# sidward14/gan-lab

Hardware: AMD Instinct MI355X
Metric: images/sec (G+D step), StyleGAN 1024^2 bs32/GPU (higher is better)
Workload: dtype f32; 1 GPU; StyleGAN res_samples=1024 FFHQ-shaped synthetic, bs=32/GPU fp32, nonsaturating + R1(lambda=10) + drift, stabilised phase, 1 D-iter + 1 G-iter; global_batch=32, per_gpu_batch=32, parallelism=single

## Files before the change

### gan_lab_amd/_lib.py

```python
import ctypes
import os
import subprocess

import torch

_HERE = os.path.dirname(os.path.abspath(__file__))
CSRC = os.path.join(_HERE, 'csrc')
SO_PATH = os.path.join(CSRC, os.path.basename(os.environ.get('GANLAB_HIP_LIB', '') or 'libganlab_hip.so'))

_c_int, _c_ll, _c_f, _c_p, _c_sz, _c_u64 = (ctypes.c_int, ctypes.c_longlong, ctypes.c_float, ctypes.c_void_p,
                                             ctypes.c_size_t, ctypes.c_uint64)
_c_d = ctypes.c_double

ACT_NONE, ACT_LRELU = 0, 1
PACK_FWD, PACK_DGRAD = 0, 1


class ConvGeom(ctypes.Structure):
    _fields_ = [('N', _c_int), ('Cin', _c_int), ('Hin', _c_int), ('Win', _c_int),
                ('Cout', _c_int), ('ks', _c_int), ('pad', _c_int), ('up', _c_int), ('pool', _c_int)]


_GP = ctypes.POINTER(ConvGeom)

# ... 1 lines not shown
class PackDesc(ctypes.Structure):
    _fields_ = [('src', _c_p), ('dst', _c_p), ('kind', _c_int), ('Cout', _c_int), ('Cin', _c_int), ('ks', _c_int),
                ('mode', _c_int), ('up', _c_int), ('scale', _c_f), ('reserved', _c_int), ('total', _c_ll),
                ('block0', _c_ll)]

class SnJob(ctypes.Structure):
    _fields_ = [('w', _c_p), ('w_sn', _c_p), ('g_sn', _c_p), ('gw', _c_p), ('u', _c_p), ('v', _c_p), ('sigma', _c_p),
                ('tpart', _c_p), ('s', _c_p), ('dpart', _c_p), ('R', _c_int), ('K', _c_int), ('blk_t0', _c_ll),
                ('blk_s0', _c_ll), ('blk_e0', _c_ll)]


SN_ROW_CHUNK, SN_COL_TILE, SN_ELEM_BLOCK = 16, 1024, 2048


class OrthoJob(ctypes.Structure):
    _fields_ = [('w', _c_p), ('gw', _c_p), ('s', _c_p), ('q', _c_p), ('part', _c_p), ('penalty', _c_p), ('R', _c_int),
                ('K', _c_int), ('form', _c_int), ('n_part', _c_int), ('blk_g0', _c_ll), ('blk_a0', _c_ll)]


class EwmaJob(ctypes.Structure):
    _fields_ = [('dst', _c_p), ('src', _c_p), ('count', _c_ll)]


ORTHO_TILE, ORTHO_QROWS, ORTHO_ROW, ORTHO_COL = 64, 4, 0, 1


class HierJob(ctypes.Structure):
    _fields_ = [('w', _c_p), ('gw', _c_p), ('gw_own', _c_p), ('C', _c_int), ('z_off', _c_int), ('z_len', _c_int),
                ('col', _c_int), ('scale', _c_f), ('one', _c_f), ('blk_f0', _c_ll), ('blk_w0', _c_ll)]


SIGNATURES = {
    'ganlab_abi_version': (_c_int, []),
    'ganlab_last_launch': (_c_int, [ctypes.c_char_p, _c_int, ctypes.POINTER(ctypes.c_uint)]),
    'ganlab_launch_count': (ctypes.c_ulonglong, []),
    'ganlab_launch_history': (_c_int, [_c_int, ctypes.c_char_p, _c_int, ctypes.POINTER(ctypes.c_uint)]),
    'ganlab_conv_geom_size': (_c_int, []),
    'ganlab_conv_out_hw': (_c_int, [_GP, ctypes.POINTER(_c_int), ctypes.POINTER(_c_int)]),
    'ganlab_conv_pack_f32': (_c_ll, [_c_p, _c_p, _c_int, _c_int, _c_int, _c_int, _c_f, _c_p]),
    'ganlab_conv_fwd_f32': (_c_int, [_c_p, _c_p, _c_p, _c_p, _GP, _c_f, _c_int, _c_f, _c_p]),
    'ganlab_conv_dgrad_f32': (_c_int, [_c_p, _c_p, _c_p, _GP, _c_p]),
    'ganlab_conv_splitk_plan': (_c_int, [_GP, _c_int]),
    'ganlab_conv_fwd_splitk_f32': (_c_int, [_c_p, _c_p, _c_p, _c_p, _GP, _c_f, _c_int, _c_f, _c_p, _c_sz, _c_p]),
    'ganlab_conv_dgrad_splitk_f32': (_c_int, [_c_p, _c_p, _c_p, _GP, _c_p, _c_sz, _c_p]),
    'ganlab_conv_dgrad_mask_supported': (_c_int, [_GP]),
    'ganlab_conv_dgrad_mask_f32': (_c_int, [_c_p, _c_p, _c_p, _c_p, _GP, _c_f, _c_p]),
    'ganlab_conv_act_bwd_fused_supported': (_c_int, [_GP]),
    'ganlab_conv_dgrad_act_f32': (_c_int, [_c_p, _c_p, _c_p, _c_p, _GP, _c_f, _c_p]),
    'ganlab_conv_fwd_mask_f32': (_c_int, [_c_p, _c_p, _c_p, _c_p, _GP, _c_f, _c_p]),
    'ganlab_conv_wgrad_act_f32': (_c_int, [_c_p, _c_p, _c_p, _c_p, _c_p, _GP, _c_f, _c_f, _c_f, _c_p, _c_sz, _c_p]),
    'ganlab_conv_wgrad_workspace': (_c_sz, [_GP]),
    'ganlab_conv_wgrad_f32': (_c_int, [_c_p, _c_p, _c_p, _GP, _c_f, _c_p, _c_sz, _c_p]),
    'ganlab_conv_s2_supported': (_c_int, [_GP]),
    'ganlab_conv_s2_pack_f32': (_c_ll, [_c_p, _c_p, _c_int, _c_int, _c_int, _c_int, _c_f, _c_p]),
    'ganlab_conv_s2_fwd_f32': (_c_int, [_c_p, _c_p, _c_p, _c_p, _GP, _c_f, _c_int, _c_f, _c_p]),
    'ganlab_conv_s2_dgrad_f32': (_c_int, [_c_p, _c_p, _c_p, _GP, _c_p]),
    'ganlab_conv_s2_wgrad_workspace': (_c_sz, [_GP]),
    'ganlab_conv_s2_wgrad_f32': (_c_int, [_c_p, _c_p, _c_p, _GP, _c_f, _c_p, _c_sz, _c_p]),
    'ganlab_conv_bf16_supported': (_c_int, [_GP]),
    'ganlab_conv_pack_bf16': (_c_ll, [_c_p, _c_p, _c_int, _c_int, _c_int, _c_f, _c_p]),
    'ganlab_conv_fwd_bf16': (_c_int, [_c_p, _c_p, _c_p, _c_p, _GP, _c_f, _c_int, _c_f, _c_p]),
    'ganlab_conv_dgrad_bf16': (_c_int, [_c_p, _c_p, _c_p, _GP, _c_p]),
    'ganlab_conv_bf16_splitk_plan': (_c_int, [_GP, _c_int]),
    'ganlab_conv_fwd_bf16_splitk': (_c_int, [_c_p, _c_p, _c_p, _c_p, _GP, _c_f, _c_int, _c_f, _c_p, _c_sz, _c_p]),
    'ganlab_conv_dgrad_bf16_splitk': (_c_int, [_c_p, _c_p, _c_p, _GP, _c_p, _c_sz, _c_p]),
    'ganlab_conv_wgrad_bf16_workspace': (_c_sz, [_GP]),
    'ganlab_conv_wgrad_bf16': (_c_int, [_c_p, _c_p, _c_p, _GP, _c_f, _c_p, _c_sz, _c_p]),
    'ganlab_conv_x3_supported': (_c_int, [_GP, _c_int]),
    'ganlab_conv_x3_pack': (_c_ll, [_c_p, _c_p, _c_int, _c_int, _c_int, _c_f, _c_p]),
    'ganlab_conv_fwd_x3': (_c_int, [_c_p, _c_p, _c_p, _c_p, _GP, _c_f, _c_int, _c_f, _c_p]),
    'ganlab_conv_dgrad_x3': (_c_int, [_c_p, _c_p, _c_p, _GP, _c_p]),
    'ganlab_conv_dgrad_mask_x3': (_c_int, [_c_p, _c_p, _c_p, _c_p, _GP, _c_f, _c_p]),
    'ganlab_conv_fwd_aff_x3': (_c_int, [_c_p, _c_p, _c_p, _c_p, _c_p, _c_p, _GP, _c_f, _c_int, _c_f, _c_p]),
    'ganlab_conv_fwd_aff_tail_x3_chunks': (_c_int, [_GP]),
    'ganlab_conv_s2_x3_supported': (_c_int, [_GP, _c_int]),
    'ganlab_conv_s2_x3_pack': (_c_ll, [_c_p, _c_p, _c_int, _c_int, _c_int, _c_f, _c_p]),
    'ganlab_conv_s2_fwd_x3': (_c_int, [_c_p, _c_p, _c_p, _c_p, _GP, _c_f, _c_int, _c_f, _c_p]),
    'ganlab_conv_s2_fwd_aff_x3': (_c_int, [_c_p, _c_p, _c_p, _c_p, _c_p, _c_p, _GP, _c_f, _c_int, _c_f, _c_p]),
    'ganlab_conv_s2_dgrad_x3': (_c_int, [_c_p, _c_p, _c_p, _GP, _c_p]),
    'ganlab_conv_s2_down_x3_supported': (_c_int, [_GP, _c_int]),
    'ganlab_conv_s2_down_x3_pack': (_c_ll, [_c_p, _c_p, _c_int, _c_int, _c_int, _c_f, _c_p]),
    'ganlab_conv_s2_down_fwd_x3': (_c_int, [_c_p, _c_p, _c_p, _c_p, _GP, _c_f, _c_int, _c_f, _c_p]),
    'ganlab_conv_s2_down_dgrad_x3': (_c_int, [_c_p, _c_p, _c_p, _GP, _c_p]),
    'ganlab_conv_wgrad_x3_supported': (_c_int, [_GP]),
    'ganlab_conv_wgrad_x3_workspace': (_c_sz, [_GP]),
    'ganlab_conv_wgrad_x3': (_c_int, [_c_p, _c_p, _c_p, _c_p, _c_p, _GP, _c_f, _c_p, _c_sz, _c_p]),
    'ganlab_conv_s2_wgrad_x3_supported': (_c_int, [_GP]),
    'ganlab_conv_s2_wgrad_x3_workspace': (_c_sz, [_GP]),
    'ganlab_conv_s2_wgrad_x3': (_c_int, [_c_p, _c_p, _c_p, _c_p, _c_p, _GP, _c_f, _c_p, _c_sz, _c_p]),
    'ganlab_conv_fwd_aff_tail_x3': (_c_int, [_c_p, _c_p, _c_p, _c_p, _c_p, _c_p, _c_p, _c_p, _c_p, _c_p, _GP, _c_f, _c_int, _c_f,
                                             _c_f, _c_p, _c_sz, _c_p]),
    'ganlab_mask_bits_supported': (_c_int, [_c_int, _c_int]),
    'ganlab_blur3x3_bits_f32': (_c_int, [_c_p, _c_p, _c_p, _c_ll, _c_int, _c_int, _c_p]),
    'ganlab_blur_act_bwd_bits_f32': (_c_int, [_c_p, _c_p, _c_p, _c_p, _c_int, _c_int, _c_int, _c_int, _c_f, _c_f,
                                              _c_p, _c_sz, _c_p]),
    'ganlab_act_bwd_blur_bits_f32': (_c_int, [_c_p, _c_p, _c_p, _c_p, _c_p, _c_p, _c_int, _c_int, _c_int, _c_int,
                                              _c_f, _c_f, _c_p, _c_sz, _c_p]),
    'ganlab_conv_fwd_blur_supported': (_c_int, [_GP, _c_p, _c_p]),
    'ganlab_conv_fwd_blur_bits_f32': (_c_int, [_c_p, _c_p, _c_p, _c_p, _c_p, _GP, _c_f, _c_f, _c_p]),
    'ganlab_conv_s2_blur_supported': (_c_int, [_GP]),
    'ganlab_conv_s2_blur_workspace': (_c_sz, [_GP]),
    'ganlab_conv_s2_fwd_blur_tail_f32': (_c_int, [_c_p, _c_p, _c_p, _c_p, _c_p, _c_p, _c_p, _c_p, _c_p, _c_p, _GP, _c_f, _c_int,
                                                  _c_f, _c_f, _c_p, _c_sz, _c_p]),
    'ganlab_conv_s2_dgrad_blur_act_bits_f32': (_c_int, [_c_p, _c_p, _c_p, _c_p, _c_p, _GP, _c_f, _c_f, _c_p, _c_sz, _c_p]),
    'ganlab_conv_dgrad_rgb_sums_supported': (_c_int, [_GP, _c_int]),
    'ganlab_conv_dgrad_rgb_sums_workspace': (_c_sz, [_GP]),
    'ganlab_conv_dgrad_rgb_sums_f32': (_c_int, [_c_p, _c_p, _c_p, _c_p, _c_p, _c_p, _GP, _c_int, _c_f, _c_f, _c_f, _c_int, _c_int,
                                                _c_p, _c_sz, _c_p]),
    'ganlab_conv_fwd_bits_f32': (_c_int, [_c_p, _c_p, _c_p, _c_p, _c_p, _GP, _c_f, _c_int, _c_f, _c_p]),
    'ganlab_conv_dgrad_act_bits_f32': (_c_int, [_c_p, _c_p, _c_p, _c_p, _GP, _c_f, _c_p]),
    'ganlab_conv_fwd_mask_bits_f32': (_c_int, [_c_p, _c_p, _c_p, _c_p, _GP, _c_f, _c_p]),
    'ganlab_conv_wgrad_act_bits_f32': (_c_int, [_c_p, _c_p, _c_p, _c_p, _c_p, _GP, _c_f, _c_f, _c_f, _c_p, _c_sz, _c_p]),
    'ganlab_pack_desc_size': (_c_int, []),
    'ganlab_pack_many': (_c_int, [_c_p, _c_int, _c_ll, _c_p]),
    'ganlab_in_affine_f32': (_c_int, [_c_p, _c_p, _c_p, _c_p, _c_p, _c_int, _c_int, _c_p]),
    'ganlab_conv_aff_supported': (_c_int, [_GP]),
    'ganlab_conv_fwd_aff_f32': (_c_int, [_c_p, _c_p, _c_p, _c_p, _c_p, _c_p, _GP, _c_f, _c_int, _c_f, _c_p]),
    'ganlab_conv_fwd_aff_tail_chunks': (_c_int, [_GP]),
    'ganlab_conv_fwd_aff_tail_f32': (_c_int, [_c_p, _c_p, _c_p, _c_p, _c_p, _c_p, _c_p, _c_p, _c_p, _c_p, _GP, _c_f, _c_int, _c_f,
                                              _c_f, _c_p, _c_sz, _c_p]),
    'ganlab_conv_wgrad_aff_f32': (_c_int, [_c_p, _c_p, _c_p, _c_p, _c_p, _GP, _c_f, _c_p, _c_sz, _c_p]),
    'ganlab_conv_s2_aff_supported': (_c_int, [_GP]),
    'ganlab_conv_s2_fwd_aff_f32': (_c_int, [_c_p, _c_p, _c_p, _c_p, _c_p, _c_p, _GP, _c_f, _c_int, _c_f, _c_p]),
    'ganlab_conv_s2_wgrad_aff_f32': (_c_int, [_c_p, _c_p, _c_p, _c_p, _c_p, _GP, _c_f, _c_p, _c_sz, _c_p]),
    'ganlab_mod_conv_supported': (_c_int, [_GP]),
    'ganlab_mod_conv_stat_chunks': (_c_int, [_GP]),
    'ganlab_mod_conv_fwd_f32': (_c_int, [_c_p, _c_p, _c_p, _c_p, _c_p, _c_p, _c_p, _c_p, _c_p, _c_p, _GP, _c_f, _c_int,
                                         _c_f, _c_f, _c_p, _c_sz, _c_p]),
    'ganlab_mod_torgb_prep_f32': (_c_int, [_c_p, _c_p, _c_p, _c_p, _c_p, _c_p, _c_int, _c_int, _c_int, _c_f, _c_f, _c_p]),
    'ganlab_mod_torgb_wgrad_f32': (_c_int, [_c_p, _c_p, _c_p, _c_p, _c_p, _c_int, _c_int, _c_int, _c_f, _c_f, _c_p]),
    'ganlab_mod_torgb_fwd_f32': (_c_int, [_c_p, _c_p, _c_p, _c_p, _c_int, _c_int, _c_int, _c_ll, _c_p]),
    'ganlab_mod_torgb_cross_workspace': (_c_sz, [_c_int]),
    'ganlab_mod_torgb_cross_f32': (_c_int, [_c_p, _c_p, _c_p, _c_int, _c_int, _c_int, _c_ll, _c_p, _c_sz, _c_p]),
    'ganlab_blur3x3_f32': (_c_int, [_c_p, _c_p, _c_ll, _c_int, _c_int, _c_p]),
    'ganlab_up2_f32': (_c_int, [_c_p, _c_p, _c_ll, _c_int, _c_int, _c_f, _c_p]),
    'ganlab_pool2_f32': (_c_int, [_c_p, _c_p, _c_ll, _c_int, _c_int, _c_f, _c_p]),
    'ganlab_resample2d_f32': (_c_int, [_c_p, _c_p, _c_p, _c_p, _c_p, _c_p, _c_ll, _c_int, _c_int, _c_int, _c_int, _c_int,
                                       _c_int, _c_p]),
    'ganlab_bias_act_f32': (_c_int, [_c_p, _c_p, _c_p, _c_p, _c_p, _c_int, _c_int, _c_ll, _c_f, _c_int, _c_f, _c_p]),
    'ganlab_act_bwd_f32': (_c_int, [_c_p, _c_p, _c_p, _c_ll, _c_f, _c_p]),
    'ganlab_act_bwd_bias_f32': (_c_int, [_c_p, _c_p, _c_p, _c_p, _c_int, _c_int, _c_ll, _c_f, _c_f, _c_p, _c_sz, _c_p]),
    'ganlab_channel_sum_f32': (_c_int, [_c_p, _c_p, _c_p, _c_int, _c_int, _c_ll, _c_f, _c_p, _c_sz, _c_p]),
    'ganlab_channel_sum_workspace': (_c_sz, [_c_int, _c_int, _c_ll]),
    'ganlab_instnorm_stats_f32': (_c_int, [_c_p, _c_p, _c_p, _c_ll, _c_ll, _c_f, _c_p]),
    'ganlab_row_stats_workspace': (_c_sz, [_c_ll, _c_ll]),
    'ganlab_row_stats_f32': (_c_int, [_c_p, _c_p, _c_p, _c_ll, _c_ll, _c_f, _c_p, _c_sz, _c_p]),
    'ganlab_instnorm_style_fwd_f32': (_c_int, [_c_p, _c_p, _c_p, _c_p, _c_p, _c_int, _c_int, _c_ll, _c_p]),
    'ganlab_instnorm_style_bwd_reduce_f32': (_c_int, [_c_p, _c_p, _c_p, _c_p, _c_p, _c_p, _c_ll, _c_ll, _c_p]),
    'ganlab_instnorm_style_bwd_apply_f32': (_c_int, [_c_p, _c_p, _c_p, _c_p, _c_p, _c_p, _c_p, _c_p, _c_int, _c_int,
                                                     _c_ll, _c_p]),
    'ganlab_pixelnorm_fwd_f32': (_c_int, [_c_p, _c_p, _c_int, _c_int, _c_ll, _c_f, _c_p]),
    'ganlab_pixelnorm_bwd_f32': (_c_int, [_c_p, _c_p, _c_p, _c_int, _c_int, _c_ll, _c_f, _c_p]),
    'ganlab_blur_fused_supported': (_c_int, [_c_int, _c_int]),
    'ganlab_blur_fused_workspace': (_c_sz, [_c_int, _c_int, _c_int, _c_int]),
    'ganlab_blur_bias_act_f32': (_c_int, [_c_p, _c_p, _c_p, _c_p, _c_p, _c_int, _c_int, _c_int, _c_int, _c_f,
                                          _c_int, _c_f, _c_p]),
    'ganlab_blur_act_bwd_f32': (_c_int, [_c_p, _c_p, _c_p, _c_p, _c_int, _c_int, _c_int, _c_int, _c_f, _c_f,
                                         _c_p, _c_sz, _c_p]),
    'ganlab_act_bwd_blur_f32': (_c_int, [_c_p, _c_p, _c_p, _c_p, _c_p, _c_p, _c_int, _c_int, _c_int, _c_int,
                                         _c_f, _c_f, _c_p, _c_sz, _c_p]),
    'ganlab_act_stats_workspace': (_c_sz, [_c_int, _c_int, _c_ll]),
    'ganlab_bias_act_stats_f32': (_c_int, [_c_p, _c_p, _c_p, _c_p, _c_p, _c_p, _c_p, _c_int, _c_int, _c_ll, _c_f, _c_int,
                                           _c_f, _c_f, _c_p, _c_sz, _c_p]),
    'ganlab_blur_bias_act_stats_f32': (_c_int, [_c_p, _c_p, _c_p, _c_p, _c_p, _c_p, _c_p, _c_int, _c_int, _c_int, _c_int,
                                                _c_f, _c_int, _c_f, _c_f, _c_p, _c_sz, _c_p]),
    'ganlab_instnorm_bwd_act_workspace': (_c_sz, [_c_int, _c_int, _c_ll]),
    'ganlab_instnorm_style_bwd_act_f32': (_c_int, [_c_p] * 11 + [_c_int, _c_int, _c_ll, _c_int, _c_f, _c_f, _c_p, _c_sz,
                                                                 _c_p]),
    'ganlab_instnorm_bwd_rgb_supported': (_c_int, [_c_int, _c_int, _c_int, _c_ll]),
    'ganlab_instnorm_bwd_reduce_rgb_workspace': (_c_sz, [_c_int, _c_int, _c_ll]),
    'ganlab_instnorm_style_bwd_reduce_rgb_f32': (_c_int, [_c_p, _c_p, _c_int] + [_c_p] * 5 + [_c_int, _c_int, _c_ll, _c_p,
                                                                                            _c_sz, _c_p]),
    'ganlab_instnorm_style_bwd_act_rgb_f32': (_c_int, [_c_p, _c_p, _c_int] + [_c_p] * 10 + [_c_int, _c_int, _c_ll, _c_int,
                                                                                         _c_f, _c_f, _c_p, _c_sz, _c_p]),
    'ganlab_instnorm_style_bwd_act_blur_f32': (_c_int, [_c_p] * 11 + [_c_int, _c_int, _c_int, _c_int, _c_int, _c_f, _c_f,
                                                                      _c_p, _c_sz, _c_p]),
    'ganlab_u8_box_decode_f32': (_c_int, [_c_p, _c_p, _c_int, _c_int, _c_int, _c_int, _c_int, _c_p, _c_p, _c_p, _c_p]),
    'ganlab_chan_affine_f32': (_c_int, [_c_p, _c_p, _c_p, _c_p, _c_int, _c_int, _c_ll, _c_p]),
    'ganlab_mul_f32': (_c_int, [_c_p, _c_p, _c_p, _c_ll, _c_p]),
    'ganlab_ln_affine_fwd_f32': (_c_int, [_c_p, _c_p, _c_p, _c_p, _c_p, _c_p, _c_int, _c_ll, _c_int, _c_f, _c_p]),
    'ganlab_colscale_f32': (_c_int, [_c_p, _c_p, _c_p, _c_int, _c_ll, _c_p]),
    'ganlab_coldot_f32': (_c_int, [_c_p, _c_p, _c_p, _c_p, _c_p, _c_p, _c_int, _c_ll, _c_p]),
    'ganlab_ln_rowsums_workspace': (_c_sz, [_c_int, _c_ll]),
    'ganlab_ln_rowsums_f32': (_c_int, [_c_p, _c_p, _c_p, _c_p, _c_p, _c_p, _c_p, _c_p, _c_int, _c_ll, _c_p, _c_sz, _c_p, _c_p,
                                       _c_f, _c_p]),
    'ganlab_ln_project_f32': (_c_int, [_c_p, _c_p, _c_p, _c_p, _c_p, _c_p, _c_p, _c_p, _c_int, _c_ll, _c_p]),
    'ganlab_ln_bwd_cols_f32': (_c_int, [_c_p, _c_p, _c_p, _c_p, _c_p, _c_p, _c_p, _c_p, _c_p, _c_int, _c_ll, _c_p]),
    'ganlab_ln_bwdbwd_apply_f32': (_c_int, [_c_p, _c_p, _c_p, _c_p, _c_p, _c_p, _c_p, _c_p, _c_int, _c_ll, _c_p]),
    'ganlab_bn_stats_f32': (_c_int, [_c_p, _c_p, _c_int, _c_int, _c_ll, _c_p, _c_sz, _c_p]),
    'ganlab_bn_finalize_f32': (_c_int, [_c_p, _c_p, _c_p, _c_p, _c_p, _c_p, _c_int, _c_f, _c_f, _c_f, _c_p]),
    'ganlab_bn_apply_f32': (_c_int, [_c_p, _c_p, _c_p, _c_p, _c_p, _c_int, _c_int, _c_ll, _c_int, _c_f, _c_p]),
    'ganlab_bn_bwd_sums_f32': (_c_int, [_c_p, _c_p, _c_p, _c_p, _c_p, _c_int, _c_int, _c_ll, _c_p, _c_sz, _c_p, _c_p, _c_f,
                                        _c_p]),
    'ganlab_bn_bwd_apply_f32': (_c_int, [_c_p, _c_p, _c_p, _c_p, _c_p, _c_p, _c_p, _c_int, _c_int, _c_ll, _c_p]),
    'ganlab_tanh_fwd_f32': (_c_int, [_c_p, _c_p, _c_ll, _c_p]),
    'ganlab_tanh_bwd_f32': (_c_int, [_c_p, _c_p, _c_p, _c_ll, _c_p]),
    'ganlab_mbstd_fwd_f32': (_c_int, [_c_p, _c_p, _c_int, _c_int, _c_ll, _c_f, _c_p]),
    'ganlab_mbstd_bwd_f32': (_c_int, [_c_p, _c_p, _c_p, _c_int, _c_int, _c_ll, _c_f, _c_p]),
    'ganlab_mbstd_bwdbwd_f32': (_c_int, [_c_p, _c_p, _c_p, _c_p, _c_p, _c_int, _c_int, _c_ll, _c_f, _c_p]),
    'ganlab_axpby_f32': (_c_int, [_c_p, _c_p, _c_p, _c_ll, _c_f, _c_f, _c_p]),
    'ganlab_scale_dev_f32': (_c_int, [_c_p, _c_p, _c_p, _c_ll, _c_f, _c_p]),
    'ganlab_lerp_rows_f32': (_c_int, [_c_p, _c_p, _c_p, _c_p, _c_ll, _c_ll, _c_p]),
    'ganlab_sum_f32': (_c_int, [_c_p, _c_p, _c_ll, _c_f, _c_int, _c_p, _c_sz, _c_p]),
    'ganlab_sum_workspace': (_c_sz, [_c_ll]),
    'ganlab_bce_logits_fwd_f32': (_c_int, [_c_p, _c_p, _c_int, _c_f, _c_p]),
    'ganlab_bce_logits_bwd_f32': (_c_int, [_c_p, _c_p, _c_p, _c_int, _c_f, _c_p]),
    'ganlab_hinge_fwd_f32': (_c_int, [_c_p, _c_p, _c_int, _c_f, _c_f, _c_p]),
    'ganlab_hinge_bwd_f32': (_c_int, [_c_p, _c_p, _c_p, _c_int, _c_f, _c_f, _c_p]),
    'ganlab_chnorm_penalty_fwd_f32': (_c_int, [_c_p, _c_p, _c_int, _c_int, _c_ll, _c_f, _c_f, _c_p, _c_sz, _c_p]),
    'ganlab_chnorm_penalty_bwd_f32': (_c_int, [_c_p, _c_p, _c_p, _c_int, _c_int, _c_ll, _c_f, _c_f, _c_p]),
    'ganlab_adam_f32': (_c_int, [_c_p, _c_p, _c_p, _c_p, _c_ll, _c_f, _c_f, _c_f, _c_f, _c_f, _c_f, _c_f, _c_p]),
    'ganlab_ewma_f32': (_c_int, [_c_p, _c_p, _c_ll, _c_f, _c_p]),
    'ganlab_randn_f32': (_c_int, [_c_p, _c_ll, _c_u64, _c_u64, _c_p]),
    'ganlab_randn_dev_f32': (_c_int, [_c_p, _c_ll, _c_u64, _c_p, _c_u64, _c_p]),
    'ganlab_diffaug_params_f32': (_c_int, [_c_p, _c_int, _c_int, _c_int, _c_u64, _c_u64, _c_p]),
    'ganlab_diffaug_params_dev_f32': (_c_int, [_c_p, _c_int, _c_int, _c_int, _c_u64, _c_p, _c_u64, _c_p]),
    'ganlab_diffaug_fwd_workspace': (_c_sz, [_c_int, _c_int, _c_int, _c_int]),
    'ganlab_diffaug_bwd_workspace': (_c_sz, [_c_int, _c_int, _c_int, _c_int]),
    'ganlab_diffaug_fwd_f32': (_c_int, [_c_p, _c_p, _c_p, _c_int, _c_int, _c_int, _c_int, _c_p, _c_sz, _c_p]),
    'ganlab_diffaug_bwd_f32': (_c_int, [_c_p, _c_p, _c_p, _c_int, _c_int, _c_int, _c_int, _c_p, _c_sz, _c_p]),
    'ganlab_ada_params_f32': (_c_int, [_c_p, _c_int, _c_int, _c_int, _c_p, _c_int, _c_u64, _c_u64, _c_p]),
    'ganlab_ada_params_dev_f32': (_c_int, [_c_p, _c_int, _c_int, _c_int, _c_p, _c_int, _c_u64, _c_p, _c_u64, _c_p]),
    'ganlab_ada_fwd_f32': (_c_int, [_c_p, _c_p, _c_p, _c_int, _c_int, _c_int, _c_p]),
    'ganlab_ada_bwd_f32': (_c_int, [_c_p, _c_p, _c_p, _c_int, _c_int, _c_int, _c_p]),
    'ganlab_ada_update_f32': (_c_int, [_c_p, _c_p, _c_int, _c_int, _c_f, _c_f, _c_p]),
    'ganlab_ada_filter_bank': (_c_int, [_c_p]),
    'ganlab_ada_ext_params_f32': (_c_int, [_c_p, _c_int, _c_int, _c_int, _c_p, _c_int, _c_u64, _c_u64, _c_p]),
    'ganlab_ada_ext_params_dev_f32': (_c_int, [_c_p, _c_int, _c_int, _c_int, _c_p, _c_int, _c_u64, _c_p, _c_u64, _c_p]),
    'ganlab_ada_ext_fwd_f32': (_c_int, [_c_p, _c_p, _c_p, _c_p, _c_int, _c_int, _c_int, _c_p]),
    'ganlab_ada_ext_bwd_f32': (_c_int, [_c_p, _c_p, _c_p, _c_int, _c_int, _c_int, _c_p]),
    'ganlab_swd_down_f32': (_c_int, [_c_p, _c_p, _c_ll, _c_int, _c_int, _c_p]),
    'ganlab_swd_band_f32': (_c_int, [_c_p, _c_p, _c_p, _c_ll, _c_int, _c_int, _c_p]),
    'ganlab_swd_gather_f32': (_c_int, [_c_p, _c_p, _c_p, _c_p, _c_int, _c_int, _c_int, _c_p]),
    'ganlab_swd_stats_f64': (_c_int, [_c_p, _c_ll, _c_ll, _c_p, _c_p]),
    'ganlab_swd_project_f32': (_c_int, [_c_p, _c_p, _c_p, _c_p, _c_ll, _c_int, _c_p]),
    'ganlab_swd_sort_workspace': (_c_sz, [_c_int, _c_ll]),
    'ganlab_swd_sort_f32': (_c_int, [_c_p, _c_p, _c_int, _c_ll, _c_p, _c_sz, _c_p]),
    'ganlab_swd_distance_workspace': (_c_sz, [_c_int, _c_ll]),
    'ganlab_swd_distance_f64': (_c_int, [_c_p, _c_p, _c_p, _c_int, _c_ll, _c_p, _c_sz, _c_p]),
    'ganlab_swd_positions_i32': (_c_int, [_c_p, _c_int, _c_int, _c_int, _c_u64, _c_u64, _c_p]),
    'ganlab_swd_directions_f32': (_c_int, [_c_p, _c_int, _c_u64, _c_u64, _c_p]),
    'ganlab_msssim_workspace': (_c_sz, [_c_int, _c_int]),
    'ganlab_msssim_level_f32': (_c_int, [_c_p, _c_p, _c_ll, _c_p, _c_p, _c_ll, _c_int, _c_int, _c_int, _c_int, _c_int, _c_f, _c_f,
                                         _c_p, _c_sz, _c_p]),
    'ganlab_msssim_finish_f64': (_c_int, [_c_p, _c_sz, _c_int, _c_int, _c_p, _c_p, _c_p, _c_p]),
    'ganlab_spectrum_workspace': (_c_sz, [_c_int, _c_int]),
    'ganlab_spectrum_scratch': (_c_sz, [_c_int, _c_int]),
    'ganlab_spectrum_feed_f32': (_c_int, [_c_p, _c_ll, _c_int, _c_int, _c_int, _c_int, _c_int, _c_p, _c_sz, _c_p, _c_sz, _c_p]),
    'ganlab_spectrum_finish_f64': (_c_int, [_c_p, _c_p, _c_sz, _c_int, _c_int, _c_p, _c_sz, _c_p]),
    'ganlab_adam_dev_f32': (_c_int, [_c_p, _c_p, _c_p, _c_p, _c_ll, _c_p, _c_f, _c_f, _c_f, _c_f, _c_p]),
    'ganlab_sn_job_size': (_c_int, []),
    'ganlab_sn_refresh': (_c_int, [_c_p, _c_int, _c_ll, _c_ll, _c_ll, _c_int, _c_f, _c_p]),
    'ganlab_sn_backward': (_c_int, [_c_p, _c_int, _c_ll, _c_p]),
    'ganlab_ortho_job_size': (_c_int, []),
    'ganlab_ortho_apply': (_c_int, [_c_p, _c_int, _c_ll, _c_ll, _c_f, _c_p, _c_p]),
    'ganlab_attn_supported': (_c_int, [_c_int, _c_int, _c_int, _c_int, _c_int]),
    'ganlab_attn_fwd_f32': (_c_int, [_c_p, _c_p, _c_p, _c_p, _c_p, _c_int, _c_int, _c_int, _c_int, _c_int, _c_p]),
    'ganlab_attn_bwd_workspace': (_c_sz, [_c_int, _c_int]),
    'ganlab_attn_bwd_f32': (_c_int, [_c_p] * 9 + [_c_int, _c_int, _c_int, _c_int, _c_int, _c_p, _c_sz, _c_p]),
    'ganlab_maxpool2x2_bits_bytes': (_c_sz, [_c_ll, _c_int, _c_int]),
    'ganlab_maxpool2x2_f32': (_c_int, [_c_p, _c_p, _c_p, _c_ll, _c_int, _c_int, _c_p]),
    'ganlab_maxpool2x2_bwd_f32': (_c_int, [_c_p, _c_p, _c_p, _c_ll, _c_int, _c_int, _c_p]),
    'ganlab_gated_residual_f32': (_c_int, [_c_p, _c_p, _c_p, _c_p, _c_ll, _c_p]),
    'ganlab_dot_workspace': (_c_sz, [_c_ll]),
    'ganlab_dot_f32': (_c_int, [_c_p, _c_p, _c_p, _c_ll, _c_p, _c_sz, _c_p]),
    'ganlab_cbn_apply_f32': (_c_int, [_c_p] * 7 + [_c_int, _c_int, _c_ll, _c_int, _c_int, _c_f, _c_p]),
    'ganlab_cbn_bwd_workspace': (_c_sz, [_c_int, _c_int]),
    'ganlab_cbn_bwd_f32': (_c_int, [_c_p] * 12 + [_c_int, _c_int, _c_ll, _c_int, _c_int, _c_f, _c_p, _c_sz, _c_p]),
    'ganlab_hier_job_size': (_c_int, []),
    'ganlab_hier_fwd_f32': (_c_int, [_c_p, _c_int, _c_ll, _c_p, _c_p, _c_p, _c_p, _c_int, _c_ll, _c_int, _c_int, _c_int, _c_p]),
    'ganlab_hier_bwd_f32': (_c_int, [_c_p, _c_int, _c_ll] + [_c_p] * 7 + [_c_int, _c_ll, _c_int, _c_int, _c_int, _c_int, _c_p]),
    'ganlab_trunc_randn_f32': (_c_int, [_c_p, _c_ll, _c_f, _c_u64, _c_u64, _c_p]),
    'ganlab_ewma_job_size': (_c_int, []),
    'ganlab_ewma_many_f32': (_c_int, [_c_p, _c_int, _c_f, _c_p]),
    'ganlab_mbn_apply_f32': (_c_int, [_c_p, _c_p, _c_p, _c_p, _c_ll, _c_p, _c_ll, _c_p, _c_int, _c_int, _c_ll, _c_int, _c_f,
                                      _c_p]),
    'ganlab_mbn_bwd_workspace': (_c_sz, [_c_int, _c_int]),
    'ganlab_mbn_bwd_f32': (_c_int, [_c_p] * 5 + [_c_ll] + [_c_p] * 5 + [_c_ll, _c_p, _c_int, _c_int, _c_ll, _c_int, _c_f, _c_p,
                                    _c_sz, _c_p]),
    'ganlab_proj_fwd_f32': (_c_int, [_c_p, _c_p, _c_p, _c_p, _c_p, _c_int, _c_ll, _c_int, _c_p]),
    'ganlab_proj_dfeat_f32': (_c_int, [_c_p, _c_p, _c_p, _c_p, _c_int, _c_ll, _c_int, _c_p]),
    'ganlab_proj_dweight_f32': (_c_int, [_c_p, _c_p, _c_p, _c_p, _c_int, _c_ll, _c_int, _c_p]),
    'ganlab_randint_i32': (_c_int, [_c_p, _c_ll, _c_int, _c_u64, _c_u64, _c_p]),
    'ganlab_prdc_norms_f32': (_c_int, [_c_p, _c_p, _c_ll, _c_int, _c_p]),
    'ganlab_prdc_knn_f32': (_c_int, [_c_p, _c_p, _c_p, _c_ll, _c_int, _c_int, _c_p]),
    'ganlab_prdc_cross_f32': (_c_int, [_c_p] * 5 + [_c_int, _c_p, _c_p, _c_p, _c_ll, _c_ll, _c_int, _c_p]),
    'ganlab_cr_params_i32': (_c_int, [_c_p, _c_int, _c_int, _c_int, _c_u64, _c_u64, _c_p, _c_p]),
    'ganlab_cr_transform_f32': (_c_int, [_c_p, _c_p, _c_p, _c_int, _c_int, _c_int, _c_int, _c_p]),
    'ganlab_cr_msd_fwd_f32': (_c_int, [_c_p, _c_p, _c_p, _c_int, _c_p]),
    'ganlab_cr_msd_bwd_f32': (_c_int, [_c_p, _c_p, _c_p, _c_p, _c_p, _c_int, _c_p]),
    'ganlab_cr_imsd_workspace': (_c_sz, [_c_ll]),
    'ganlab_cr_imsd_fwd_f32': (_c_int, [_c_p, _c_p, _c_p, _c_ll, _c_p, _c_sz, _c_p]),
    'ganlab_cr_imsd_bwd_f32': (_c_int, [_c_p, _c_p, _c_p, _c_p, _c_p, _c_ll, _c_p]),
    'ganlab_moments_accum_f32': (_c_int, [_c_p, _c_ll, _c_int, _c_p, _c_p, _c_p, _c_p]),
    'ganlab_kid_rowsums_f32': (_c_int, [_c_p, _c_ll, _c_p, _c_ll, _c_int, _c_f, _c_f, _c_int, _c_p, _c_p]),
    'ganlab_class_ce_fwd_f32': (_c_int, [_c_p, _c_p, _c_p, _c_p, _c_int, _c_int, _c_p]),
    'ganlab_class_ce_bwd_f32': (_c_int, [_c_p, _c_p, _c_p, _c_p, _c_p, _c_int, _c_int, _c_p]),
    'ganlab_cl_supported': (_c_int, [_c_int, _c_int, _c_int]),
    'ganlab_cl_fwd_f32': (_c_int, [_c_p] * 5 + [_c_int, _c_int, _c_int, _c_int, _c_f, _c_f, _c_f, _c_p]),
    'ganlab_cl_bwd_workspace': (_c_sz, [_c_int, _c_int, _c_int]),
    'ganlab_cl_bwd_f32': (_c_int, [_c_p] * 7 + [_c_int, _c_int, _c_int, _c_int, _c_f, _c_f, _c_f, _c_p, _c_sz, _c_p]),
    'ganlab_pyramid_mse_workspace': (_c_sz, [_c_int, _c_int, _c_int, _c_int]),
    'ganlab_pyramid_mse_f32': (_c_int, [_c_p] * 3 + [_c_int] + [_c_p] * 3 + [_c_int, _c_int, _c_int, _c_p, _c_sz, _c_p]),
    'ganlab_scale_rows_f32': (_c_int, [_c_p, _c_p, _c_p, _c_int, _c_ll, _c_p]),
    'ganlab_w_moments_workspace': (_c_sz, [_c_int]),
    'ganlab_w_moments_f32': (_c_int, [_c_p, _c_p, _c_p, _c_ll, _c_int, _c_p, _c_sz, _c_p]),
    'ganlab_project_step_f32': (_c_int, [_c_p] * 8 + [_c_int, _c_int, _c_int, _c_int, _c_p, _c_p]),
    'ganlab_step_scalars_size': (_c_int, []),
    'ganlab_set_step_scalars': (_c_int, [_c_p, _c_u64, _c_f, _c_f, _c_f, _c_f, _c_f, _c_f, _c_p]),
    'ganlab_ppl_endpoints_f32': (_c_int, [_c_p, _c_p, _c_p, _c_p, _c_ll, _c_int, _c_d, _c_int, _c_int, _c_u64, _c_u64, _c_p]),
    'ganlab_row_sqdist_f32': (_c_int, [_c_p, _c_p, _c_p, _c_ll, _c_ll, _c_p]),
    'ganlab_trimmed_mean_workspace': (_c_sz, [_c_ll]),
    'ganlab_trimmed_mean_f32': (_c_int, [_c_p, _c_ll, _c_d, _c_d, _c_p, _c_p, _c_sz, _c_p]),
}

_LIB = None


class GanlabLibraryError(RuntimeError):
    pass


def build(verbose=False):
    res = subprocess.run(['make', '-C', CSRC, '-j4'], capture_output=True, text=True)
    if verbose or res.returncode != 0:
        print(res.stdout)
        print(res.stderr)
    if res.returncode != 0:
        raise GanlabLibraryError('building libganlab_hip.so failed:\n' + res.stderr[-4000:])
    return SO_PATH


def lib():
    global _LIB
    if _LIB is None:
        if not os.path.exists(SO_PATH):
            raise GanlabLibraryError(
                f'{SO_PATH} not found: the HIP kernel library is required (there is no CPU/PyTorch '
                f'fallback). Build it with `python -c "import __graft_entry__ as g; g.build()"` or '
                f'`make -C {CSRC}`.')
        handle = ctypes.CDLL(SO_PATH)
        for name, (res, args) in SIGNATURES.items():
            fn = getattr(handle, name)
            fn.restype = res
            fn.argtypes = args
        if handle.ganlab_conv_geom_size() != ctypes.sizeof(ConvGeom):
            raise GanlabLibraryError(f'ConvGeom mirror is {ctypes.sizeof(ConvGeom)} bytes, the library\'s '
                                     f'ganlab_conv_geom {handle.ganlab_conv_geom_size()}: header and binding disagree')
        if handle.ganlab_pack_desc_size() != ctypes.sizeof(PackDesc):
            raise GanlabLibraryError(f'PackDesc mirror is {ctypes.sizeof(PackDesc)} bytes, the library\'s '
                                     f'ganlab_pack_desc {handle.ganlab_pack_desc_size()}: header and binding disagree')
        if handle.ganlab_sn_job_size() != ctypes.sizeof(SnJob):
            raise GanlabLibraryError(f'SnJob mirror is {ctypes.sizeof(SnJob)} bytes, the library\'s '
                                     f'ganlab_sn_job {handle.ganlab_sn_job_size()}: header and binding disagree')
        if handle.ganlab_ortho_job_size() != ctypes.sizeof(OrthoJob):
            raise GanlabLibraryError(f'OrthoJob mirror is {ctypes.sizeof(OrthoJob)} bytes, the library\'s '
                                     f'ganlab_ortho_job {handle.ganlab_ortho_job_size()}: header and binding disagree')
        if handle.ganlab_hier_job_size() != ctypes.sizeof(HierJob):
            raise GanlabLibraryError(f'HierJob mirror is {ctypes.sizeof(HierJob)} bytes, the library\'s '
                                     f'ganlab_hier_job {handle.ganlab_hier_job_size()}: header and binding disagree')
        if handle.ganlab_ewma_job_size() != ctypes.sizeof(EwmaJob):
            raise GanlabLibraryError(f'EwmaJob mirror is {ctypes.sizeof(EwmaJob)} bytes, the library\'s '
                                     f'ganlab_ewma_job {handle.ganlab_ewma_job_size()}: header and binding disagree')
        _LIB = handle
    return _LIB


def last_launch():
    buf = ctypes.create_string_buffer(1024)
    grid = ctypes.c_uint(0)
    n = lib().ganlab_last_launch(buf, 1024, ctypes.byref(grid))
    return (buf.value.decode() if n > 0 else None), int(grid.value)


def launch_count():
    return int(lib().ganlab_launch_count())


def launches_since(count):
    n = min(launch_count() - count, 16)
    out = []
    buf = ctypes.create_string_buffer(1024)
    grid = ctypes.c_uint(0)
    for back in range(n - 1, -1, -1):
        if lib().ganlab_launch_history(back, buf, 1024, ctypes.byref(grid)) > 0:
            out.append((buf.value.decode(), int(grid.value)))
    return out


_ERR = {-1: 'GANLAB_EINVAL (bad argument)', -2: 'GANLAB_EWORKSPACE (workspace too small)',
        -3: 'GANLAB_ELAUNCH (kernel launch failed)', -4: 'GANLAB_EUNSUPPORTED (geometry not handled)'}


def check(rc, what):
    if rc != 0:
        raise GanlabLibraryError(f'{what} failed: {_ERR.get(rc, rc)}')
```

### gan_lab_amd/_ops/pointwise.py

```python
import numpy as np

import torch
from torch.autograd import Function
from torch.autograd.function import once_differentiable

from .. import _lib
from .._lib import check
from .core import _c, _nchw, _new, _p, _st, _take


def k_blur(x):
    x = _c(x)
    n, c, h, w = x.shape
    y = torch.empty_like(x)
    check(_lib.lib().ganlab_blur3x3_f32(_p(x), _p(y), n * c, h, w, _st()), 'blur3x3')
    return y


def decode_u8(images_u8_nhwc, res, mean, std, flip=None):
    x = images_u8_nhwc
    if not x.is_cuda or x.dtype != torch.uint8 or x.dim() != 4:
        raise TypeError('decode_u8 needs a (N,H,W,C) uint8 tensor on the GPU')
    x = x.contiguous()
    n, hs, ws, c = x.shape
    if hs % res or ws % res or hs // res != ws // res:
        raise ValueError(f'cannot box-resize {hs}x{ws} to {res}x{res}')
    mean = torch.as_tensor(mean, dtype=torch.float32, device=x.device).contiguous()
    std = torch.as_tensor(std, dtype=torch.float32, device=x.device).contiguous()
    assert mean.numel() == c and std.numel() == c
    if flip is not None:
        flip = flip.to(device=x.device, dtype=torch.uint8).contiguous()
        assert flip.numel() == n
    out = torch.empty((n, c, res, res), dtype=torch.float32, device=x.device)
    check(_lib.lib().ganlab_u8_box_decode_f32(x.data_ptr(), _p(out), n, hs, ws, c, hs // res, _p(mean), _p(std),
                                              flip.data_ptr() if flip is not None else None, _st()), 'u8_box_decode')
    return out


def k_up2(x, scale=1.0):
    x = _c(x)
    n, c, h, w = x.shape
    y = _new((n, c, 2 * h, 2 * w), x)
    check(_lib.lib().ganlab_up2_f32(_p(x), _p(y), n * c, h, w, scale, _st()), 'up2')
    return y


def k_pool2(x, scale=0.25):
    x = _c(x)
    n, c, h, w = x.shape
    assert h % 2 == 0 and w % 2 == 0
    y = _new((n, c, h // 2, w // 2), x)
    check(_lib.lib().ganlab_pool2_f32(_p(x), _p(y), n * c, h // 2, w // 2, scale, _st()), 'pool2')
    return y


RESAMPLE_MODES = ('bilinear_up', 'bilinear_down', 'nearest_down')


_RESAMPLE_TABLES = {}


def resample_matrix(mode, align_corners, n_in):
    if mode not in RESAMPLE_MODES:
        raise ValueError(f'resampler mode {mode!r}: one of {RESAMPLE_MODES}')
    f32 = np.float32
    n_out = 2 * n_in if mode == 'bilinear_up' else n_in // 2
    if n_out < 1 or (mode != 'bilinear_up' and n_in % 2):
        raise ValueError(f'{mode}: size {n_in} has no 0.5x / 2x counterpart')
    m = np.zeros((n_out, n_in), np.float64)
    inv = f32(0.5) if mode == 'bilinear_up' else f32(2.0)
    for o in range(n_out):
        if mode == 'nearest_down':
            m[o, min(int(np.floor(f32(o) * inv)), n_in - 1)] = 1.0
            continue
        if align_corners:
            r = f32(n_in - 1) / f32(n_out - 1) if n_out > 1 else f32(0)
            src = r * f32(o)
        else:
            src = max(inv * (f32(o) + f32(0.5)) - f32(0.5), f32(0))
        i0 = min(int(src), n_in - 1)
        i1 = i0 + (1 if i0 < n_in - 1 else 0)
        l1 = f32(src) - f32(i0)
        m[o, i0] += float(f32(1) - l1)
        m[o, i1] += float(l1)
    return m


def _taps(m):
    nz = [np.nonzero(row)[0] for row in m]
    t = max(1, max(len(v) for v in nz))
    if t > 6:
        raise ValueError(f'resampler needs {t} taps per output (the kernel holds 6)')
    idx, w = np.zeros((m.shape[0], t), np.int32), np.zeros((m.shape[0], t), np.float32)
    for o, v in enumerate(nz):
        idx[o, :len(v)] = v
        w[o, :len(v)] = m[o, v]
    return idx, w, t


def _resample_tables(mode, align, n_in, adjoint, device):
    key = (mode, bool(align), int(n_in), bool(adjoint), str(device))
    tab = _RESAMPLE_TABLES.get(key)
    if tab is None:
        m = resample_matrix(mode, align, n_in)
        idx, w, t = _taps(m.T if adjoint else m)
        tab = (torch.from_numpy(idx).to(device), torch.from_numpy(w).to(device), t, idx.shape[0])
        _RESAMPLE_TABLES[key] = tab
    return tab


def k_resample(x, mode, align, hin, win, adjoint):
    x = _c(x)
    n, c, h, w = x.shape
    iy, wy, ty, ho = _resample_tables(mode, align, hin, adjoint, x.device)
    ix, wx, tx, wo = _resample_tables(mode, align, win, adjoint, x.device)
    exp_h = hin if not adjoint else (2 * hin if mode == 'bilinear_up' else hin // 2)
    exp_w = win if not adjoint else (2 * win if mode == 'bilinear_up' else win // 2)
    if (h, w) != (exp_h, exp_w):
        raise ValueError(f'resample {mode} (adjoint={adjoint}): input {h}x{w}, expected {exp_h}x{exp_w}')
    y = _new((n, c, ho, wo), x)
    check(_lib.lib().ganlab_resample2d_f32(_p(x), _p(y), _p(iy), _p(wy), _p(ix), _p(wx), n * c, h, w, ho, wo, ty, tx,
                                           _st()), 'resample2d')
    return y


def k_bias_act(x, bias, noise, noise_w, bias_scale, act, slope):
    x = _c(x)
    n, c, hw = _nchw(x)
    y = torch.empty_like(x)
    bias = _c(bias) if bias is not None else None
    noise = _c(noise) if noise is not None else None
    noise_w = _c(noise_w) if noise_w is not None else None
    if noise is not None:
        assert noise.numel() == n * hw and noise_w.numel() == c
    check(_lib.lib().ganlab_bias_act_f32(_p(x), _p(bias), _p(noise), _p(noise_w), _p(y), n, c, hw, bias_scale, act,
                                         slope, _st()), 'bias_act')
    return y


def k_act_bwd(gy, y, slope):
    gy, y = _c(gy), _c(y)
    assert gy.shape == y.shape
    gz = torch.empty_like(gy)
    check(_lib.lib().ganlab_act_bwd_f32(_p(gy), _p(y), _p(gz), gy.numel(), slope, _st()), 'act_bwd')
    return gz


def k_act_bwd_bias(gy, y, slope, scale):
    gy, y = _c(gy), _c(y)
    assert gy.shape == y.shape
    n, c, hw = _nchw(gy)
    L = _lib.lib()
    ws = torch.empty((L.ganlab_channel_sum_workspace(n, c, hw) + 3) // 4, dtype=torch.float32, device=gy.device)
    gz, gb = torch.empty_like(gy), _take('gb', (c,), gy)
    check(L.ganlab_act_bwd_bias_f32(_p(gy), _p(y), _p(gz), _p(gb), n, c, hw, slope, scale, _p(ws), ws.numel() * 4,
                                    _st()), 'act_bwd_bias')
    return gz, gb


def k_channel_sum(a, b=None, scale=1.0, sink=None):
    a = _c(a)
# ... 331 lines not shown
```

### gan_lab_amd/csrc/pointwise.hip

```cpp
#include "common.h"

#include <stdlib.h>

namespace {

constexpr int kMaxBlocks = 256 * 8;

inline unsigned ew_blocks(long long n_items) {
  long long b = (n_items + 255) / 256;
  if (b < 1) b = 1;
  if (b > kMaxBlocks) b = kMaxBlocks;
  return (unsigned)b;
}

struct ChunkRange { long long begin, end, stride; };
__device__ __forceinline__ ChunkRange chunk_range(long long hw4, int chunks, int c, int contig) {
  ChunkRange r;
  if (contig) {
    const long long rows = (hw4 + 255) / 256, per = (rows + chunks - 1) / chunks;
    r.begin = (long long)c * per * 256;
    r.end = r.begin + per * 256;
    if (r.end > hw4) r.end = hw4;
    r.stride = 256;
  } else {
    r.begin = (long long)c * 256;
    r.end = hw4;
    r.stride = (long long)chunks * 256;
  }
  return r;
}
inline int pw_contig() {
  static const int v = [] { const char* e = getenv("GANLAB_PW_CONTIG"); return (e && e[0] == '0') ? 0 : 1; }();
  return v;
}

#define GRID_STRIDE(i, n) \
  for (long long i = blockIdx.x * (long long)blockDim.x + threadIdx.x; i < (n); i += (long long)gridDim.x * blockDim.x)

__global__ void blur3x3_kernel(const float* __restrict__ x, float* __restrict__ y, long long planes, int H, int W) {
  const long long total = planes * H * W;
  GRID_STRIDE(i, total) {
    const int w = (int)(i % W);
    const long long t = i / W;
    const int h = (int)(t % H);
    const float* px = x + (t - h) * W;
    float acc = 0.f;
#pragma unroll
    for (int dy = -1; dy <= 1; ++dy) {
      const int yy = h + dy;
      if ((unsigned)yy >= (unsigned)H) continue;
      const float* row = px + (long long)yy * W;
      const float l = (w > 0) ? row[w - 1] : 0.f;
      const float c = row[w];
      const float r = (w + 1 < W) ? row[w + 1] : 0.f;
      const float rs = l + 2.f * c + r;
      acc += (dy == 0) ? 2.f * rs : rs;
    }
    y[i] = acc * (1.f / 16.f);
  }
}

__device__ __forceinline__ unsigned mask_nibble(const unsigned* __restrict__ bits, long long e) {
  return (bits[e >> 5] >> (unsigned)(e & 31)) & 0xFu;
}
__device__ __forceinline__ unsigned mask_bit(const unsigned* __restrict__ bits, long long e) {
  return (bits[e >> 5] >> (unsigned)(e & 31)) & 1u;
}

template <bool MASKED, bool BITS = false>
__device__ __forceinline__ void blur_row(const float* __restrict__ in, const float* __restrict__ m, long long ro,
                                         int x0, int q, int w4, bool valid, float slope, float (&hrow)[4],
                                         float (&cen)[4], const unsigned* __restrict__ mb = nullptr,
                                         long long mplane = 0) {
  float4 v = make_float4(0.f, 0.f, 0.f, 0.f);
  if (valid) {
    v = *reinterpret_cast<const float4*>(in + ro + x0);
    if (MASKED) {
      if (BITS) {
        const unsigned nb = mask_nibble(mb, mplane + ro + x0);
        v.x = (nb & 1u) ? v.x : v.x * slope;
        v.y = (nb & 2u) ? v.y : v.y * slope;
        v.z = (nb & 4u) ? v.z : v.z * slope;
        v.w = (nb & 8u) ? v.w : v.w * slope;
      } else {
        const float4 mm = *reinterpret_cast<const float4*>(m + ro + x0);
        v.x = mm.x > 0.f ? v.x : v.x * slope;
        v.y = mm.y > 0.f ? v.y : v.y * slope;
        v.z = mm.z > 0.f ? v.z : v.z * slope;
        v.w = mm.w > 0.f ? v.w : v.w * slope;
      }
    }
  }
  const int lane = threadIdx.x & 63;
  float l = __shfl_up(v.w, 1, 64);
  float r = __shfl_down(v.x, 1, 64);
  const bool need_l = lane == 0 && q != 0, need_r = lane == 63 && q != w4 - 1;
  float e = 0.f;
  if (valid && (need_l || need_r)) {
    const long long eo = ro + x0 + (need_l ? -1 : 4);
    e = in[eo];
    if (MASKED) {
      if (BITS) e = mask_bit(mb, mplane + eo) ? e : e * slope;
      else e = m[eo] > 0.f ? e : e * slope;
    }
  }
  if (q == 0) l = 0.f;
  else if (lane == 0) l = e;
  if (q == w4 - 1) r = 0.f;
  else if (lane == 63) r = e;
  hrow[0] = l + 2.f * v.x + v.y;
  hrow[1] = v.x + 2.f * v.y + v.z;
  hrow[2] = v.y + 2.f * v.z + v.w;
  hrow[3] = v.z + 2.f * v.w + r;
  cen[0] = v.x; cen[1] = v.y; cen[2] = v.z; cen[3] = v.w;
}

template <int R, bool BITS = false>
__global__ __launch_bounds__(256) void blur3x3_vec_kernel(const float* __restrict__ x, float* __restrict__ y,
                                                          long long planes, int H, int W,
                                                          unsigned* __restrict__ bits = nullptr) {
  const int w4 = W >> 2, hr = H / R;
  const long long total = planes * hr * w4;
  const long long span = (long long)gridDim.x * blockDim.x;
  for (long long base = blockIdx.x * (long long)blockDim.x; base < total; base += span) {
    const long long i = base + threadIdx.x;
    const bool live = i < total;
    const long long ii = live ? i : total - 1;
    const int q = (int)(ii % w4);
    const long long t = ii / w4;
    const int rr = (int)(t % hr);
    const long long pl = t / hr;
    const float* px = x + pl * H * W;
    const int y0 = R * rr, x0 = 4 * q;
    float h[R + 2][4], cen[4];
    [[maybe_unused]] unsigned nib[R];
#pragma unroll
    for (int k = 0; k < R + 2; ++k) {
      const int yy = y0 - 1 + k;
      blur_row<false>(px, nullptr, (long long)yy * W, x0, q, w4, (unsigned)yy < (unsigned)H, 0.f, h[k], cen);
      if constexpr (BITS) {
        if (k >= 1 && k <= R)
          nib[k - 1] = (cen[0] > 0.f ? 1u : 0u) | (cen[1] > 0.f ? 2u : 0u) | (cen[2] > 0.f ? 4u : 0u) | (cen[3] > 0.f ? 8u : 0u);
      }
    }
    if constexpr (BITS) {
      const int sh = 4 * (threadIdx.x & 7);
#pragma unroll
      for (int k = 0; k < R; ++k) {
        unsigned wv = nib[k] << sh;
        wv |= __shfl_xor(wv, 1, 64);
        wv |= __shfl_xor(wv, 2, 64);
        wv |= __shfl_xor(wv, 4, 64);
        if (live && (threadIdx.x & 7) == 0) bits[(pl * H * W + (long long)(y0 + k) * W + x0) >> 5] = wv;
      }
    }
    if (live) {
      float* py = y + pl * H * W + (long long)y0 * W + x0;
#pragma unroll
      for (int k = 0; k < R; ++k) {
        float4 o;
        o.x = (h[k][0] + 2.f * h[k + 1][0] + h[k + 2][0]) * 0.0625f;
        o.y = (h[k][1] + 2.f * h[k + 1][1] + h[k + 2][1]) * 0.0625f;
        o.z = (h[k][2] + 2.f * h[k + 1][2] + h[k + 2][2]) * 0.0625f;
        o.w = (h[k][3] + 2.f * h[k + 1][3] + h[k + 2][3]) * 0.0625f;
        *reinterpret_cast<float4*>(py + (long long)k * W) = o;
      }
    }
  }
}

__global__ void up2_kernel(const float* __restrict__ x, float* __restrict__ y, long long planes, int H, int W,
                           float scale) {
  const int Wo = 2 * W, Ho = 2 * H;
  const long long total = planes * Ho * Wo;
  GRID_STRIDE(i, total) {
    const int w = (int)(i % Wo);
    const long long t = i / Wo;
    const int h = (int)(t % Ho);
    const long long pl = t / Ho;
    y[i] = scale * x[(pl * H + (h >> 1)) * W + (w >> 1)];
  }
}

__global__ void pool2_kernel(const float* __restrict__ x, float* __restrict__ y, long long planes, int Ho, int Wo,
                             float scale) {
  const int W = 2 * Wo;
  const long long total = planes * Ho * Wo;
  GRID_STRIDE(i, total) {
    const int w = (int)(i % Wo);
    const long long t = i / Wo;
    const float2 a = *reinterpret_cast<const float2*>(x + (2 * t) * W + 2 * w);
    const float2 b = *reinterpret_cast<const float2*>(x + (2 * t + 1) * W + 2 * w);
    y[i] = scale * ((a.x + a.y) + (b.x + b.y));
  }
}

enum { BF_FWD = 0, BF_A = 1, BF_AT = 2 };

template <int MODE, int R, bool STATS = false, bool BITS = false>
__global__ __launch_bounds__(256) void blur_fused_kernel(const float* __restrict__ in, const float* __restrict__ y,
                                                         const float* __restrict__ noise,
                                                         const float* __restrict__ bias,
                                                         const float* __restrict__ noise_w, float* __restrict__ out,
                                                         double* __restrict__ part, int N, int C, int H, int W,
                                                         int chunks, float bias_scale, int act, float slope,
                                                         int want_sums, double* __restrict__ spart = nullptr) {
  __shared__ double red[4];
  __shared__ double dred[2][4];
  const int c = blockIdx.y, chunk = blockIdx.x;
  const int w4 = W >> 2, hr = H / R;
  const long long per_n = (long long)hr * w4, total = STATS ? per_n : (long long)N * per_n, HW = (long long)H * W;
  double ds = 0.0, dss = 0.0;
  const float b = (MODE == BF_FWD && bias) ? bias[c] * bias_scale : 0.f;
  const float nw = (MODE == BF_FWD && noise) ? noise_w[c] : 0.f;
  double s0 = 0.0, s1 = 0.0;
  for (long long base = chunk * 256LL; base < total; base += (long long)chunks * 256) {
    const long long i = base + threadIdx.x;
    const bool live = i < total;
    const long long ii = live ? i : total - 1;
    const long long n = STATS ? (long long)blockIdx.z : ii / per_n, rem = STATS ? ii : ii - n * per_n;
    const int rr = (int)(rem / w4), q = (int)(rem - (long long)rr * w4);
    const long long plane = (n * C + c) * HW;
    const int y0 = R * rr, x0 = 4 * q;
    float h[R + 2][4], cen[R + 2][4];
#pragma unroll
    for (int k = 0; k < R + 2; ++k) {
      const int yy = y0 - 1 + k;
      blur_row<MODE == BF_AT, BITS>(in + plane, (MODE == BF_AT && !BITS) ? y + plane : nullptr, (long long)yy * W, x0, q,
                                    w4, (unsigned)yy < (unsigned)H, slope, h[k], cen[k],
                                    reinterpret_cast<const unsigned*>(y), plane);
    }
    if (!live) continue;
    const long long co = (long long)y0 * W + x0;
#pragma unroll
    for (int k = 0; k < R; ++k) {
      float o[4];
#pragma unroll
      for (int j = 0; j < 4; ++j) o[j] = (h[k][j] + 2.f * h[k + 1][j] + h[k + 2][j]) * 0.0625f;
      if (MODE == BF_FWD) {
        float nz[4] = {0.f, 0.f, 0.f, 0.f};
        if (noise) *reinterpret_cast<float4*>(nz) = *reinterpret_cast<const float4*>(noise + n * HW + co + k * W);
#pragma unroll
        for (int j = 0; j < 4; ++j) {
          float t = o[j] + b + nw * nz[j];
          if (act == GANLAB_ACT_LRELU) t = gl_lrelu(t, slope);
          o[j] = t;
          if (STATS) {
            const double d = (double)t;
            ds += d;
            dss += d * d;
          }
        }
      } else if (MODE == BF_A) {
        if constexpr (BITS) {
          const unsigned nb = mask_nibble(reinterpret_cast<const unsigned*>(y), plane + co + (long long)k * W);
#pragma unroll
          for (int j = 0; j < 4; ++j) {
            o[j] = ((nb >> j) & 1u) ? o[j] : o[j] * slope;
            s0 += (double)o[j];
          }
        } else {
          float m[4];
          *reinterpret_cast<float4*>(m) = *reinterpret_cast<const float4*>(y + plane + co + k * W);
#pragma unroll
          for (int j = 0; j < 4; ++j) {
            o[j] = m[j] > 0.f ? o[j] : o[j] * slope;
            s0 += (double)o[j];
          }
        }
      } else {
        float nz[4] = {0.f, 0.f, 0.f, 0.f};
        if (noise && want_sums)
          *reinterpret_cast<float4*>(nz) = *reinterpret_cast<const float4*>(noise + n * HW + co + k * W);
#pragma unroll
        for (int j = 0; j < 4; ++j) {
          s0 += (double)cen[k + 1][j];
          s1 += (double)cen[k + 1][j] * nz[j];
        }
      }
      *reinterpret_cast<float4*>(out + plane + co + (long long)k * W) = *reinterpret_cast<float4*>(o);
    }
  }
  if (STATS) {
#pragma unroll
    for (int o = 32; o > 0; o >>= 1) {
      ds += __shfl_xor(ds, o, 64);
      dss += __shfl_xor(dss, o, 64);
    }
    if ((threadIdx.x & 63) == 0) {
      dred[0][threadIdx.x >> 6] = ds;
      dred[1][threadIdx.x >> 6] = dss;
    }
    __syncthreads();
    if (threadIdx.x < 2) {
      const int k = threadIdx.x;
      spart[(((long long)blockIdx.z * C + c) * chunks + chunk) * 2 + k] = (dred[k][0] + dred[k][1]) + (dred[k][2] + dred[k][3]);
    }
  }
  if (MODE != BF_FWD && want_sums) {
    s0 = gl_block_sum_256d(s0, red);
    if (threadIdx.x == 0) part[(long long)c * chunks + chunk] = s0;
    if (MODE == BF_AT) {
      __syncthreads();
      s1 = gl_block_sum_256d(s1, red);
      if (threadIdx.x == 0) part[((long long)C + c) * chunks + chunk] = s1;
    }
  }
}

template <int R>
__global__ __launch_bounds__(256) void instnorm_bwd_act_blur_kernel(
    const float* __restrict__ gy, const float* __restrict__ x, const float* __restrict__ mean,
    const float* __restrict__ rstd, const float* __restrict__ style, const float* __restrict__ s1,
    const float* __restrict__ s2, const float* __restrict__ noise, float* __restrict__ out, double* __restrict__ part,
    int N, int C, int H, int W, int chunks, int act, float slope, int want_b, int want_nw) {
  __shared__ double red[4];
  const int c = blockIdx.y, n = blockIdx.z, chunk = blockIdx.x;
  const long long pl = (long long)n * C + c, HW = (long long)H * W;
  const int w4 = W >> 2, hr = H / R;
  const long long per_n = (long long)hr * w4;
  const double md = (double)mean[pl], rd = (double)rstd[pl];
  const double ys = style ? (double)style[((long long)n * 2 + 0) * C + c] + 1.0 : 1.0;
  const double inv = 1.0 / (double)HW;
  const double k = rd * ys, a1 = (double)s1[pl] * inv, a2 = (double)s2[pl] * inv;
  const float* pg = gy + pl * HW;
  const float* px = x + pl * HW;
  const float* pn = (want_nw && noise) ? noise + (long long)n * HW : nullptr;
  float* po = out + pl * HW;
  const int lane = threadIdx.x & 63;
  double sb = 0.0, snw = 0.0;
  auto zval = [&](float g, float v) -> double {
    double t = k * ((double)g - a1 - ((double)v - md) * rd * a2);
    if (act == GANLAB_ACT_LRELU && !(v > 0.f)) t *= (double)slope;
    return t;
  };
  for (long long base = chunk * 256LL; base < per_n; base += (long long)chunks * 256) {
    const long long i = base + threadIdx.x;
    const bool live = i < per_n;
    const long long ii = live ? i : per_n - 1;
    const int rr = (int)(ii / w4), q = (int)(ii - (long long)rr * w4);
    const int y0 = R * rr, x0 = 4 * q;
    float h[R + 2][4];
#pragma unroll
    for (int kk = 0; kk < R + 2; ++kk) {
      const int yy = y0 - 1 + kk;
      const bool valid = (unsigned)yy < (unsigned)H;
      const long long ro = (long long)yy * W;
      float z[4] = {0.f, 0.f, 0.f, 0.f};
      if (valid) {
        float g[4], v[4];
        *reinterpret_cast<float4*>(g) = *reinterpret_cast<const float4*>(pg + ro + x0);
        *reinterpret_cast<float4*>(v) = *reinterpret_cast<const float4*>(px + ro + x0);
        const bool own = live && kk >= 1 && kk <= R;
        float nz[4] = {0.f, 0.f, 0.f, 0.f};
        if (own && pn) *reinterpret_cast<float4*>(nz) = *reinterpret_cast<const float4*>(pn + ro + x0);
#pragma unroll
        for (int j = 0; j < 4; ++j) {
          const double t = zval(g[j], v[j]);
          z[j] = (float)t;
          if (own) {
            sb += t;
            snw += t * (double)nz[j];
          }
        }
      }
      float l = __shfl_up(z[3], 1, 64);
      float r = __shfl_down(z[0], 1, 64);
      const bool need_l = lane == 0 && q != 0, need_r = lane == 63 && q != w4 - 1;
      float e = 0.f;
      if (valid && (need_l || need_r)) {
        const long long eo = ro + x0 + (need_l ? -1 : 4);
        e = (float)zval(pg[eo], px[eo]);
      }
      if (q == 0) l = 0.f;
      else if (lane == 0) l = e;
      if (q == w4 - 1) r = 0.f;
      else if (lane == 63) r = e;
      h[kk][0] = l + 2.f * z[0] + z[1];
      h[kk][1] = z[0] + 2.f * z[1] + z[2];
      h[kk][2] = z[1] + 2.f * z[2] + z[3];
      h[kk][3] = z[2] + 2.f * z[3] + r;
    }
    if (!live) continue;
#pragma unroll
    for (int kk = 0; kk < R; ++kk) {
      float4 o;
      o.x = (h[kk][0] + 2.f * h[kk + 1][0] + h[kk + 2][0]) * 0.0625f;
      o.y = (h[kk][1] + 2.f * h[kk + 1][1] + h[kk + 2][1]) * 0.0625f;
      o.z = (h[kk][2] + 2.f * h[kk + 1][2] + h[kk + 2][2]) * 0.0625f;
      o.w = (h[kk][3] + 2.f * h[kk + 1][3] + h[kk + 2][3]) * 0.0625f;
      *reinterpret_cast<float4*>(po + (long long)(y0 + kk) * W + x0) = o;
    }
  }
  const long long slot = ((long long)c * N + n) * chunks + chunk;
  if (want_b) {
    sb = gl_block_sum_256d(sb, red);
    if (threadIdx.x == 0) part[slot] = sb;
  }
  if (want_nw) {
    if (want_b) __syncthreads();
    snw = gl_block_sum_256d(snw, red);
    if (threadIdx.x == 0) part[(long long)C * N * chunks + slot] = snw;
  }
}

inline int blur_rows(int H) { return (H & 3) == 0 ? 4 : 2; }
inline int blur_rows_mode(int H, int mode) {
  const int min8 = mode == BF_FWD ? 512 : (mode == BF_A ? 256 : (1 << 30));
  return ((H & 7) == 0 && H >= min8) ? 8 : blur_rows(H);
}
#define BLUR_FUSED_LAUNCH(MODE, ...)                                                                   \
  do {                                                                                                 \
    const int rows_ = blur_rows_mode(H, MODE);                                                         \
    if (rows_ == 8) GL_LAUNCH((blur_fused_kernel<MODE, 8>), dim3(chunks, C), dim3(256), 0, ST, __VA_ARGS__);      \
    else if (rows_ == 4) GL_LAUNCH((blur_fused_kernel<MODE, 4>), dim3(chunks, C), dim3(256), 0, ST, __VA_ARGS__); \
    else GL_LAUNCH((blur_fused_kernel<MODE, 2>), dim3(chunks, C), dim3(256), 0, ST, __VA_ARGS__);                \
  } while (0)

#define BLUR_FUSED_LAUNCH_BITS(MODE, ...)                                                                            \
  do {                                                                                                               \
    const int rows_ = blur_rows_mode(H, MODE);                                                                       \
    if (rows_ == 8) GL_LAUNCH((blur_fused_kernel<MODE, 8, false, true>), dim3(chunks, C), dim3(256), 0, ST, __VA_ARGS__);      \
    else if (rows_ == 4) GL_LAUNCH((blur_fused_kernel<MODE, 4, false, true>), dim3(chunks, C), dim3(256), 0, ST, __VA_ARGS__); \
    else GL_LAUNCH((blur_fused_kernel<MODE, 2, false, true>), dim3(chunks, C), dim3(256), 0, ST, __VA_ARGS__);                \
  } while (0)

inline int blur_fused_chunks(int N, int H, int W) {
  long long c = ((long long)N * (H / blur_rows(H)) * (W / 4) + 256 * 4 - 1) / (256 * 4);
  if (c < 1) c = 1;
  if (c > 128) c = 128;
  return (int)c;
}

__global__ __launch_bounds__(256) void bias_act_stats_kernel(const float* __restrict__ x, const float* __restrict__ bias,
                                                             const float* __restrict__ noise,
                                                             const float* __restrict__ noise_w, float* __restrict__ y,
                                                             double* __restrict__ spart, int C, long long hw4,
                                                             int chunks, float bias_scale, int act, float slope,
                                                             int contig) {
  __shared__ double dred[2][4];
  const long long pl = blockIdx.y;
  const int c = (int)(pl % C);
  const long long n = pl / C;
  const float b = bias ? bias[c] * bias_scale : 0.f;
  const float nw = noise ? noise_w[c] : 0.f;
  const float4* xp = reinterpret_cast<const float4*>(x) + pl * hw4;
  const float4* np = noise ? reinterpret_cast<const float4*>(noise) + n * hw4 : nullptr;
  float4* yp = reinterpret_cast<float4*>(y) + pl * hw4;
  double ds = 0.0, dss = 0.0;
  const ChunkRange cr = chunk_range(hw4, chunks, blockIdx.x, contig);
  for (long long i = cr.begin + threadIdx.x; i < cr.end; i += cr.stride) {
    float v[4], nz[4] = {0.f, 0.f, 0.f, 0.f};
    *reinterpret_cast<float4*>(v) = xp[i];
    if (np) *reinterpret_cast<float4*>(nz) = np[i];
#pragma unroll
    for (int k = 0; k < 4; ++k) {
      float t = v[k] + b + nw * nz[k];
      if (act == GANLAB_ACT_LRELU) t = gl_lrelu(t, slope);
      v[k] = t;
      const double d = (double)t;
      ds += d;
      dss += d * d;
    }
    yp[i] = *reinterpret_cast<float4*>(v);
  }
#pragma unroll
  for (int o = 32; o > 0; o >>= 1) {
    ds += __shfl_xor(ds, o, 64);
    dss += __shfl_xor(dss, o, 64);
  }
  if ((threadIdx.x & 63) == 0) {
    dred[0][threadIdx.x >> 6] = ds;
    dred[1][threadIdx.x >> 6] = dss;
  }
  __syncthreads();
  if (threadIdx.x < 2) {
    const int k = threadIdx.x;
    spart[(pl * chunks + blockIdx.x) * 2 + k] = (dred[k][0] + dred[k][1]) + (dred[k][2] + dred[k][3]);
  }
}

__global__ void act_stats_finish_kernel(const double* __restrict__ spart, float* __restrict__ mean,
                                        float* __restrict__ rstd, long long planes, int chunks, double inv_hw, float eps) {
  const long long pl = blockIdx.x * (long long)blockDim.x + threadIdx.x;
  if (pl >= planes) return;
  double s = 0.0, ss = 0.0;
  for (int k = 0; k < chunks; ++k) {
    s += spart[(pl * chunks + k) * 2];
    ss += spart[(pl * chunks + k) * 2 + 1];
  }
  const double m = s * inv_hw;
  double var = ss * inv_hw - m * m;
  if (var < 0.0) var = 0.0;
  mean[pl] = (float)m;
  rstd[pl] = (float)(1.0 / sqrt(var + (double)eps));
}

__global__ __launch_bounds__(256) void row_stats_partial_kernel(const float* __restrict__ x, double* __restrict__ spart,
                                                                int chunks, long long m4) {
  __shared__ double red[2][4];
  const long long row = blockIdx.x / chunks;
  const int k = blockIdx.x % chunks;
  const long long per = (m4 + chunks - 1) / chunks, lo = k * per, hi = lo + per < m4 ? lo + per : m4;
  const float4* p4 = reinterpret_cast<const float4*>(x) + row * m4;
  double s = 0.0, ss = 0.0;
  for (long long i = lo + threadIdx.x; i < hi; i += 256) {
    const float4 v = p4[i];
    const double a = (double)v.x, b = (double)v.y, c = (double)v.z, d = (double)v.w;
    s += (a + b) + (c + d);
    ss += (a * a + b * b) + (c * c + d * d);
  }
#pragma unroll
  for (int o = 32; o > 0; o >>= 1) {
    s += __shfl_xor(s, o, 64);
    ss += __shfl_xor(ss, o, 64);
  }
  if ((threadIdx.x & 63) == 0) {
    red[0][threadIdx.x >> 6] = s;
    red[1][threadIdx.x >> 6] = ss;
  }
  __syncthreads();
  if (threadIdx.x == 0) {
    spart[((long long)blockIdx.x) * 2] = (red[0][0] + red[0][1]) + (red[0][2] + red[0][3]);
    spart[((long long)blockIdx.x) * 2 + 1] = (red[1][0] + red[1][1]) + (red[1][2] + red[1][3]);
  }
}

inline int act_stats_chunks(long long hw4) {
  long long c = (hw4 + 256 * 8 - 1) / (256 * 8);
  if (c < 1) c = 1;
  if (c > 64) c = 64;
  return (int)c;
}

template <int VEC>
__global__ void bias_act_kernel(const float* __restrict__ x, const float* __restrict__ bias,
                                const float* __restrict__ noise, const float* __restrict__ noise_w,
                                float* __restrict__ y, int N, int C, long long HW, float bias_scale, int act,
                                float slope) {
  const long long hwv = HW / VEC, total = (long long)N * C * hwv;
  GRID_STRIDE(i, total) {
    const long long pl = i / hwv, hv = i - pl * hwv;
    const int c = (int)(pl % C);
    const long long n = pl / C;
    const float b = bias ? bias[c] * bias_scale : 0.f;
    const float nw = noise ? noise_w[c] : 0.f;
    float v[VEC], nz[VEC];
    if (VEC == 4) {
      *reinterpret_cast<float4*>(v) = *reinterpret_cast<const float4*>(x + i * 4);
      if (noise) *reinterpret_cast<float4*>(nz) = *reinterpret_cast<const float4*>(noise + (n * hwv + hv) * 4);
    } else {
      v[0] = x[i];
      if (noise) nz[0] = noise[n * HW + hv];
    }
#pragma unroll
    for (int k = 0; k < VEC; ++k) {
      float t = v[k] + b;
      if (noise) t += nw * nz[k];
      if (act == GANLAB_ACT_LRELU) t = gl_lrelu(t, slope);
      v[k] = t;
    }
    if (VEC == 4) *reinterpret_cast<float4*>(y + i * 4) = *reinterpret_cast<float4*>(v);
    else y[i] = v[0];
  }
}

__global__ void act_bwd_kernel(const float* __restrict__ gy, const float* __restrict__ y, float* __restrict__ gz,
                               long long n, long long n4, float slope) {
  GRID_STRIDE(i, n4) {
    const float4 g = reinterpret_cast<const float4*>(gy)[i];
    const float4 o = reinterpret_cast<const float4*>(y)[i];
    float4 r;
    r.x = o.x > 0.f ? g.x : g.x * slope;
    r.y = o.y > 0.f ? g.y : g.y * slope;
    r.z = o.z > 0.f ? g.z : g.z * slope;
    r.w = o.w > 0.f ? g.w : g.w * slope;
    reinterpret_cast<float4*>(gz)[i] = r;
  }
// ... 803 lines not shown
  __shared__ float red[4];
  double s = 0.0;
  for (int i = threadIdx.x; i < nb; i += 256) s += part[i];
  float f = gl_block_sum_256((float)s, red);
  if (threadIdx.x == 0) out[0] = f * scale;
}

inline int sum_blocks(long long n) {
  long long b = (n + 256 * 16 - 1) / (256 * 16);
  if (b < 1) b = 1;
  if (b > 1024) b = 1024;
  return (int)b;
}

__global__ __launch_bounds__(256) void bce_fwd_kernel(const float* __restrict__ x, float* __restrict__ out, int n,
                                                      float t) {
  __shared__ float red[4];
  float s = 0.f;
  for (int i = threadIdx.x; i < n; i += 256) {
    const float v = x[i];
    s += fmaxf(v, 0.f) - v * t + log1pf(expf(-fabsf(v)));
  }
  s = gl_block_sum_256(s, red);
  if (threadIdx.x == 0) out[0] = s / (float)n;
}

__global__ void bce_bwd_kernel(const float* __restrict__ x, const float* __restrict__ gout, float* __restrict__ gx,
                               int n, float t) {
  const int i = blockIdx.x * blockDim.x + threadIdx.x;
  if (i < n) {
    const float v = x[i];
    const float sg = 1.f / (1.f + expf(-v));
    gx[i] = gout[0] * (sg - t) / (float)n;
  }
}

__global__ __launch_bounds__(256) void hinge_fwd_kernel(const float* __restrict__ x, float* __restrict__ out, int n,
                                                        float a, float b) {
  __shared__ float red[4];
  float s = 0.f;
  for (int i = threadIdx.x; i < n; i += 256) s += fmaxf(a + b * x[i], 0.f);
  s = gl_block_sum_256(s, red);
  if (threadIdx.x == 0) out[0] = s / (float)n;
}

__global__ void hinge_bwd_kernel(const float* __restrict__ x, const float* __restrict__ gout, float* __restrict__ gx,
                                 int n, float a, float b) {
  const int i = blockIdx.x * blockDim.x + threadIdx.x;
  if (i < n) gx[i] = (a + b * x[i] > 0.f) ? gout[0] * b / (float)n : 0.f;
}

__global__ __launch_bounds__(256) void chnorm_pen_stage1(const float* __restrict__ g, float* __restrict__ part,
                                                         int N, int C, long long HW, float gamma) {
  __shared__ float red[4];
  const long long total = (long long)N * HW;
  float s = 0.f;
  GRID_STRIDE(i, total) {
    const long long n = i / HW, hw = i - n * HW;
    const float* p = g + n * C * HW + hw;
    float q = 0.f;
    for (int c = 0; c < C; ++c) q += p[c * HW] * p[c * HW];
    const float d = sqrtf(q) - gamma;
    s += d * d;
  }
  s = gl_block_sum_256(s, red);
  if (threadIdx.x == 0) part[blockIdx.x] = s;
}

__global__ void chnorm_pen_bwd_kernel(const float* __restrict__ g, const float* __restrict__ gout,
                                      float* __restrict__ gg, int N, int C, long long HW, float gamma, float scale) {
  const long long total = (long long)N * HW;
  const float go = gout[0] * scale * 2.f;
  GRID_STRIDE(i, total) {
    const long long n = i / HW, hw = i - n * HW;
    const float* p = g + n * C * HW + hw;
    float q = 0.f;
    for (int c = 0; c < C; ++c) q += p[c * HW] * p[c * HW];
    const float s = sqrtf(q);
    const float k = s > 0.f ? go * (s - gamma) / s : 0.f;
    float* o = gg + n * C * HW + hw;
    for (int c = 0; c < C; ++c) o[c * HW] = k * p[c * HW];
  }
}

__global__ void adam_kernel(float* __restrict__ p, const float* __restrict__ g, float* __restrict__ m,
                            float* __restrict__ v, long long n, float lr, float b1, float b2, float eps, float wd,
                            float bc1, float bc2, const float* __restrict__ dev) {
  if (dev != nullptr) {
    lr = dev[0];
    bc1 = dev[1];
    bc2 = dev[2];
  }
  const float step = lr / bc1, isq = rsqrtf(bc2);
  GRID_STRIDE(i, n) {
    float gi = g[i];
    const float pi = p[i];
    if (wd != 0.f) gi += wd * pi;
    const float mi = b1 * m[i] + (1.f - b1) * gi;
    const float vi = b2 * v[i] + (1.f - b2) * gi * gi;
    m[i] = mi;
    v[i] = vi;
    p[i] = pi - step * mi / (sqrtf(vi) * isq + eps);
  }
}

__global__ void ewma_kernel(float* __restrict__ lag, const float* __restrict__ p, long long n, float beta) {
  GRID_STRIDE(i, n) lag[i] = p[i] * (1.f - beta) + lag[i] * beta;
}

__global__ void randn_kernel(float* __restrict__ out, long long n, uint64_t seed, uint64_t offset,
                             const uint64_t* __restrict__ base) {
  if (base != nullptr) offset += *base;
  const long long n4 = (n + 3) >> 2;
  GRID_STRIDE(i, n4) {
    const uint64_t ctr = offset + (uint64_t)i;
    uint32_t c[4] = {(uint32_t)ctr, (uint32_t)(ctr >> 32), 0u, 0u};
    philox4x32_10(c, (uint32_t)seed, (uint32_t)(seed >> 32));
    float r[4];
#pragma unroll
    for (int k = 0; k < 2; ++k) {
      const float u1 = ((float)c[2 * k] + 1.0f) * (1.0f / 4294967296.0f);
      const float u2 = (float)c[2 * k + 1] * (1.0f / 4294967296.0f);
      const float rad = sqrtf(-2.f * logf(u1));
      float sn, cs;
      sincosf(6.28318530717958647692f * u2, &sn, &cs);
      r[2 * k] = rad * cs;
      r[2 * k + 1] = rad * sn;
    }
    for (int k = 0; k < 4; ++k)
      if (i * 4 + k < n) out[i * 4 + k] = r[k];
  }
}

__global__ void set_scalars_kernel(uint32_t* __restrict__ block, uint64_t rng_base, float f0, float f1, float f2,
                                   float f3, float f4, float f5) {
  if (threadIdx.x == 0 && blockIdx.x == 0) {
    *reinterpret_cast<uint64_t*>(block) = rng_base;
    float* f = reinterpret_cast<float*>(block) + 4;
    f[0] = f0; f[1] = f1; f[2] = f2; f[3] = f3; f[4] = f4; f[5] = f5;
  }
}

}

#define ST gl_stream(stream)

extern "C" {

int ganlab_abi_version(void) { return 1; }

int ganlab_blur3x3_f32(const float* x, float* y, long long planes, int H, int W, void* stream) {
  if (!x || !y || planes <= 0 || H <= 0 || W <= 0) return GANLAB_EINVAL;
  if ((W & 3) == 0 && (H & 1) == 0 && ((reinterpret_cast<uintptr_t>(x) | reinterpret_cast<uintptr_t>(y)) & 15) == 0)
    if ((H & 7) == 0 && H >= 256)
      GL_LAUNCH(blur3x3_vec_kernel<8>, dim3(ew_blocks(planes * (H / 8) * (W / 4))), dim3(256), 0, ST, x, y, planes, H,
                W);
    else if ((H & 3) == 0)
      GL_LAUNCH(blur3x3_vec_kernel<4>, dim3(ew_blocks(planes * (H / 4) * (W / 4))), dim3(256), 0, ST, x, y, planes, H,
                W);
    else
      GL_LAUNCH(blur3x3_vec_kernel<2>, dim3(ew_blocks(planes * (H / 2) * (W / 4))), dim3(256), 0, ST, x, y, planes, H,
                W);
  else
    GL_LAUNCH(blur3x3_kernel, dim3(ew_blocks(planes * H * W)), dim3(256), 0, ST, x, y, planes, H, W);
  return GL_CHECK_LAUNCH();
}

int ganlab_mask_bits_supported(int H, int W) { return (H >= 2 && (H & 1) == 0 && W >= 32 && (W & 31) == 0) ? 1 : 0; }

int ganlab_blur3x3_bits_f32(const float* x, float* y, unsigned* bits, long long planes, int H, int W, void* stream) {
  if (!x || !y || !bits || planes <= 0) return GANLAB_EINVAL;
  if (!ganlab_mask_bits_supported(H, W) || ((reinterpret_cast<uintptr_t>(x) | reinterpret_cast<uintptr_t>(y)) & 15) != 0)
    return GANLAB_EUNSUPPORTED;
  if ((H & 7) == 0 && H >= 256)
    GL_LAUNCH((blur3x3_vec_kernel<8, true>), dim3(ew_blocks(planes * (H / 8) * (W / 4))), dim3(256), 0, ST, x, y, planes, H,
              W, bits);
  else if ((H & 3) == 0)
    GL_LAUNCH((blur3x3_vec_kernel<4, true>), dim3(ew_blocks(planes * (H / 4) * (W / 4))), dim3(256), 0, ST, x, y, planes, H,
              W, bits);
  else
    GL_LAUNCH((blur3x3_vec_kernel<2, true>), dim3(ew_blocks(planes * (H / 2) * (W / 4))), dim3(256), 0, ST, x, y, planes, H,
              W, bits);
  return GL_CHECK_LAUNCH();
}

int ganlab_up2_f32(const float* x, float* y, long long planes, int H, int W, float scale, void* stream) {
  if (!x || !y || planes <= 0 || H <= 0 || W <= 0) return GANLAB_EINVAL;
  GL_LAUNCH(up2_kernel, dim3(ew_blocks(planes * H * W * 4)), dim3(256), 0, ST, x, y, planes, H, W, scale);
  return GL_CHECK_LAUNCH();
}

int ganlab_pool2_f32(const float* x, float* y, long long planes, int Hout, int Wout, float scale, void* stream) {
  if (!x || !y || planes <= 0 || Hout <= 0 || Wout <= 0) return GANLAB_EINVAL;
  GL_LAUNCH(pool2_kernel, dim3(ew_blocks(planes * Hout * Wout)), dim3(256), 0, ST, x, y, planes, Hout,
                     Wout, scale);
  return GL_CHECK_LAUNCH();
}

int ganlab_bias_act_f32(const float* x, const float* bias, const float* noise, const float* noise_w, float* y,
                        int N, int C, long long HW, float bias_scale, int act, float slope, void* stream) {
  if (!x || !y || N <= 0 || C <= 0 || HW <= 0 || (noise && !noise_w)) return GANLAB_EINVAL;
  const uintptr_t ptrs =
      reinterpret_cast<uintptr_t>(x) | reinterpret_cast<uintptr_t>(y) | reinterpret_cast<uintptr_t>(noise);
  if ((HW & 3) == 0 && (ptrs & 15) == 0)
    GL_LAUNCH(bias_act_kernel<4>, dim3(ew_blocks((long long)N * C * HW / 4)), dim3(256), 0, ST, x, bias,
                       noise, noise_w, y, N, C, HW, bias_scale, act, slope);
  else
    GL_LAUNCH(bias_act_kernel<1>, dim3(ew_blocks((long long)N * C * HW)), dim3(256), 0, ST, x, bias,
                       noise, noise_w, y, N, C, HW, bias_scale, act, slope);
  return GL_CHECK_LAUNCH();
}

int ganlab_act_bwd_f32(const float* gy, const float* y, float* gz, long long n, float slope, void* stream) {
  if (!gy || !y || !gz || n <= 0) return GANLAB_EINVAL;
  const uintptr_t ptrs = reinterpret_cast<uintptr_t>(gy) | reinterpret_cast<uintptr_t>(y) | reinterpret_cast<uintptr_t>(gz);
  if ((ptrs & 15) == 0)
    GL_LAUNCH(act_bwd_kernel, dim3(ew_blocks((n >> 2) + 4)), dim3(256), 0, ST, gy, y, gz, n, n >> 2, slope);
  else
    GL_LAUNCH(act_bwd_kernel, dim3(ew_blocks(n)), dim3(256), 0, ST, gy, y, gz, n, 0LL, slope);
  return GL_CHECK_LAUNCH();
}

size_t ganlab_channel_sum_workspace(int N, int C, long long HW) {
  return (size_t)C * channel_chunks(N, HW) * sizeof(double);
}

int ganlab_channel_sum_f32(const float* a, const float* b, float* out, int N, int C, long long HW, float scale,
                           void* workspace, size_t workspace_bytes, void* stream) {
  if (!a || !out || N <= 0 || C <= 0 || HW <= 0) return GANLAB_EINVAL;
  const int chunks = channel_chunks(N, HW);
  if (!workspace || workspace_bytes < (size_t)C * chunks * sizeof(double)) return GANLAB_EWORKSPACE;
  const int vec = ((HW & 3) == 0 && (((long long)N * HW) >> 2) < 0x7fffffffLL &&
                   ((reinterpret_cast<uintptr_t>(a) | reinterpret_cast<uintptr_t>(b)) & 15) == 0) ? 1 : 0;
  GL_LAUNCH(channel_sum_stage1, dim3(chunks, C), dim3(256), 0, ST, a, b, (double*)workspace, N, C, HW,
                     chunks, vec);
  GL_LAUNCH(channel_sum_stage2, dim3(C), dim3(64), 0, ST, (const double*)workspace, out, C, chunks, scale);
  return GL_CHECK_LAUNCH();
}

int ganlab_act_bwd_bias_f32(const float* gy, const float* y, float* gz, float* gb, int N, int C, long long HW,
                            float slope, float scale, void* workspace, size_t workspace_bytes, void* stream) {
  if (!gy || !y || !gz || !gb || N <= 0 || C <= 0 || HW <= 0) return GANLAB_EINVAL;
  const int chunks = channel_chunks(N, HW);
  if (!workspace || workspace_bytes < (size_t)C * chunks * sizeof(double)) return GANLAB_EWORKSPACE;
  GL_LAUNCH(act_bwd_bias_stage1, dim3(chunks, C), dim3(256), 0, ST, gy, y, gz, (double*)workspace, N, C, HW, chunks,
            slope);
  GL_LAUNCH(channel_sum_stage2, dim3(C), dim3(64), 0, ST, (const double*)workspace, gb, C, chunks, scale);
  return GL_CHECK_LAUNCH();
}

int ganlab_blur_fused_supported(int H, int W) { return (H >= 2 && W >= 4 && (H & 1) == 0 && (W & 3) == 0) ? 1 : 0; }

size_t ganlab_blur_fused_workspace(int N, int C, int H, int W) {
  if (!ganlab_blur_fused_supported(H, W)) return 0;
  return (size_t)2 * C * blur_fused_chunks(N, H, W) * sizeof(double);
}

int ganlab_blur_bias_act_f32(const float* x, const float* bias, const float* noise, const float* noise_w, float* y,
                             int N, int C, int H, int W, float bias_scale, int act, float slope, void* stream) {
  if (!x || !y || N <= 0 || C <= 0 || (noise && !noise_w)) return GANLAB_EINVAL;
  if (!ganlab_blur_fused_supported(H, W)) return GANLAB_EUNSUPPORTED;
  const int chunks = blur_fused_chunks(N, H, W);
  BLUR_FUSED_LAUNCH(BF_FWD, x, (const float*)nullptr, noise, bias, noise_w, y, (double*)nullptr, N, C, H, W, chunks,
                    bias_scale, act, slope, 0);
  return GL_CHECK_LAUNCH();
}

size_t ganlab_act_stats_workspace(int N, int C, long long HW) {
  if (N <= 0 || C <= 0 || HW <= 0) return 0;
  return (size_t)N * C * 128 * 2 * sizeof(double);
}

size_t ganlab_instnorm_bwd_act_workspace(int N, int C, long long HW) {
  if (N <= 0 || C <= 0 || HW <= 0) return 0;
  return (size_t)2 * N * C * 64 * sizeof(double);
}

int ganlab_instnorm_style_bwd_act_f32(const float* gy, const float* x, const float* mean, const float* rstd,
                                      const float* style, const float* s1, const float* s2, const float* noise,
                                      float* gz, float* gb, float* gnw, int N, int C, long long HW, int act,
                                      float slope, float bias_scale, void* workspace, size_t workspace_bytes,
                                      void* stream) {
  if (!gy || !x || !mean || !rstd || !s1 || !s2 || !gz || N <= 0 || C <= 0 || HW <= 0 || (gnw && !noise))
    return GANLAB_EINVAL;
  if ((HW & 3) != 0) return GANLAB_EUNSUPPORTED;
  if ((gb || gnw) && (!workspace || workspace_bytes < ganlab_instnorm_bwd_act_workspace(N, C, HW)))
    return GANLAB_EWORKSPACE;
  const long long hw4 = HW / 4, planes = (long long)N * C;
  const int chunks = act_stats_chunks(hw4);
  double* part = reinterpret_cast<double*>(workspace);
  GL_LAUNCH(instnorm_bwd_apply_act_kernel, dim3((unsigned)chunks, (unsigned)planes), dim3(256), 0, ST, gy, x, mean,
            rstd, style, s1, s2, noise, gz, part, N, C, hw4, chunks, act, slope, gb ? 1 : 0, gnw ? 1 : 0, pw_contig());
  if (gb) GL_LAUNCH(channel_sum_stage2, dim3(C), dim3(64), 0, ST, (const double*)part, gb, C, N * chunks, bias_scale);
  if (gnw)
    GL_LAUNCH(channel_sum_stage2, dim3(C), dim3(64), 0, ST, (const double*)part + (size_t)C * N * chunks, gnw, C,
              N * chunks, 1.f);
  return GL_CHECK_LAUNCH();
}

int ganlab_instnorm_bwd_rgb_supported(int N, int C, int crgb, long long HW) {
  return (N > 0 && N <= 65535 && C > 0 && C <= 16 && crgb > 0 && crgb <= 4 && HW >= 1024 && (HW & 3) == 0) ? 1 : 0;
}

static RgbSrc make_rgb_src(const float* grgb, const float* wp, int crgb, int C) {
  RgbSrc r;
  r.grgb = grgb; r.wp = wp; r.crgb = crgb; r.cout_p = (C + 63) / 64 * 64;
  return r;
}

size_t ganlab_instnorm_bwd_reduce_rgb_workspace(int N, int C, long long HW) {
  if (!ganlab_instnorm_bwd_rgb_supported(N, C, 3, HW)) return 0;
  return (size_t)N * C * act_stats_chunks(HW / 4) * 2 * sizeof(double);
}

int ganlab_instnorm_style_bwd_reduce_rgb_f32(const float* grgb, const float* wp, int crgb, const float* x,
                                             const float* mean, const float* rstd, float* s1, float* s2, int N, int C,
                                             long long HW, void* workspace, size_t workspace_bytes, void* stream) {
  if (!grgb || !wp || !x || !mean || !rstd || !s1 || !s2) return GANLAB_EINVAL;
  if (!ganlab_instnorm_bwd_rgb_supported(N, C, crgb, HW)) return GANLAB_EUNSUPPORTED;
  if (!workspace || workspace_bytes < ganlab_instnorm_bwd_reduce_rgb_workspace(N, C, HW)) return GANLAB_EWORKSPACE;
  const long long hw4 = HW / 4, planes = (long long)N * C;
  const int chunks = act_stats_chunks(hw4);
  double* part = reinterpret_cast<double*>(workspace);
  if (C == RGB_MAXC && crgb == 3)
    GL_LAUNCH(instnorm_bwd_reduce_rgb_kernel<true>, dim3((unsigned)chunks, (unsigned)N), dim3(256), 0, ST,
              make_rgb_src(grgb, wp, crgb, C), x, mean, rstd, part, C, hw4, chunks, pw_contig());
  else
    GL_LAUNCH(instnorm_bwd_reduce_rgb_kernel<false>, dim3((unsigned)chunks, (unsigned)N), dim3(256), 0, ST,
              make_rgb_src(grgb, wp, crgb, C), x, mean, rstd, part, C, hw4, chunks, pw_contig());
  GL_LAUNCH(instnorm_bwd_reduce_rgb_finish_kernel, dim3((unsigned)((planes + 63) / 64)), dim3(64), 0, ST,
            (const double*)part, s1, s2, planes, chunks);
  return GL_CHECK_LAUNCH();
}

int ganlab_instnorm_style_bwd_act_rgb_f32(const float* grgb, const float* wp, int crgb, const float* x, const float* mean,
                                          const float* rstd, const float* style, const float* s1, const float* s2,
                                          const float* noise, float* gz, float* gb, float* gnw, int N, int C, long long HW,
                                          int act, float slope, float bias_scale, void* workspace, size_t workspace_bytes,
                                          void* stream) {
  if (!grgb || !wp || !x || !mean || !rstd || !s1 || !s2 || !gz || (gnw && !noise)) return GANLAB_EINVAL;
  if (!ganlab_instnorm_bwd_rgb_supported(N, C, crgb, HW)) return GANLAB_EUNSUPPORTED;
  if ((gb || gnw) && (!workspace || workspace_bytes < ganlab_instnorm_bwd_act_workspace(N, C, HW)))
    return GANLAB_EWORKSPACE;
  const long long hw4 = HW / 4;
  const int chunks = act_stats_chunks(hw4);
  double* part = reinterpret_cast<double*>(workspace);
  if (C == RGB_MAXC && crgb == 3 && act == GANLAB_ACT_LRELU)
    GL_LAUNCH(instnorm_bwd_apply_act_rgb_kernel<true>, dim3((unsigned)chunks, (unsigned)N), dim3(256), 0, ST,
              make_rgb_src(grgb, wp, crgb, C), x, mean, rstd, style, s1, s2, noise, gz, part, N, C, hw4, chunks, act, slope,
              gb ? 1 : 0, gnw ? 1 : 0, pw_contig());
  else
    GL_LAUNCH(instnorm_bwd_apply_act_rgb_kernel<false>, dim3((unsigned)chunks, (unsigned)N), dim3(256), 0, ST,
              make_rgb_src(grgb, wp, crgb, C), x, mean, rstd, style, s1, s2, noise, gz, part, N, C, hw4, chunks, act, slope,
              gb ? 1 : 0, gnw ? 1 : 0, pw_contig());
  if (gb) GL_LAUNCH(channel_sum_stage2, dim3(C), dim3(64), 0, ST, (const double*)part, gb, C, N * chunks, bias_scale);
  if (gnw)
    GL_LAUNCH(channel_sum_stage2, dim3(C), dim3(64), 0, ST, (const double*)part + (size_t)C * N * chunks, gnw, C,
              N * chunks, 1.f);
  return GL_CHECK_LAUNCH();
}

int ganlab_instnorm_style_bwd_act_blur_f32(const float* gy, const float* x, const float* mean, const float* rstd,
                                           const float* style, const float* s1, const float* s2, const float* noise,
                                           float* out, float* gb, float* gnw, int N, int C, int H, int W, int act,
                                           float slope, float bias_scale, void* workspace, size_t workspace_bytes,
                                           void* stream) {
  if (!gy || !x || !mean || !rstd || !s1 || !s2 || !out || N <= 0 || C <= 0 || (gnw && !noise)) return GANLAB_EINVAL;
  if (!ganlab_blur_fused_supported(H, W) || N > 65535 || C > 65535) return GANLAB_EUNSUPPORTED;
  const long long HW = (long long)H * W;
  if ((gb || gnw) && (!workspace || workspace_bytes < ganlab_instnorm_bwd_act_workspace(N, C, HW))) return GANLAB_EWORKSPACE;
  const int rows = blur_rows(H);
  const long long per_n = (long long)(H / rows) * (W / 4);
  int chunks = (int)((per_n + 256 * 4 - 1) / (256 * 4));
  if (chunks < 1) chunks = 1;
  if (chunks > 64) chunks = 64;
  double* part = reinterpret_cast<double*>(workspace);
  const dim3 grid((unsigned)chunks, (unsigned)C, (unsigned)N);
  if (rows == 4)
    GL_LAUNCH(instnorm_bwd_act_blur_kernel<4>, grid, dim3(256), 0, ST, gy, x, mean, rstd, style, s1, s2, noise, out, part, N, C,
              H, W, chunks, act, slope, gb ? 1 : 0, gnw ? 1 : 0);
  else
    GL_LAUNCH(instnorm_bwd_act_blur_kernel<2>, grid, dim3(256), 0, ST, gy, x, mean, rstd, style, s1, s2, noise, out, part, N, C,
              H, W, chunks, act, slope, gb ? 1 : 0, gnw ? 1 : 0);
  if (gb) GL_LAUNCH(channel_sum_stage2, dim3(C), dim3(64), 0, ST, (const double*)part, gb, C, N * chunks, bias_scale);
  if (gnw)
    GL_LAUNCH(channel_sum_stage2, dim3(C), dim3(64), 0, ST, (const double*)part + (size_t)C * N * chunks, gnw, C,
              N * chunks, 1.f);
  return GL_CHECK_LAUNCH();
}

int ganlab_bias_act_stats_f32(const float* x, const float* bias, const float* noise, const float* noise_w, float* y,
                              float* mean, float* rstd, int N, int C, long long HW, float bias_scale, int act,
                              float slope, float eps, void* workspace, size_t workspace_bytes, void* stream) {
  if (!x || !y || !mean || !rstd || N <= 0 || C <= 0 || HW <= 0 || (noise && !noise_w)) return GANLAB_EINVAL;
  if ((HW & 3) != 0) return GANLAB_EUNSUPPORTED;
  if (!workspace || workspace_bytes < ganlab_act_stats_workspace(N, C, HW)) return GANLAB_EWORKSPACE;
  const long long hw4 = HW / 4, planes = (long long)N * C;
  const int chunks = act_stats_chunks(hw4);
  double* sp = reinterpret_cast<double*>(workspace);
  GL_LAUNCH(bias_act_stats_kernel, dim3((unsigned)chunks, (unsigned)planes), dim3(256), 0, ST, x, bias, noise, noise_w,
            y, sp, C, hw4, chunks, bias_scale, act, slope, pw_contig());
  GL_LAUNCH(act_stats_finish_kernel, dim3((unsigned)((planes + 255) / 256)), dim3(256), 0, ST, (const double*)sp, mean,
            rstd, planes, chunks, 1.0 / (double)HW, eps);
  return GL_CHECK_LAUNCH();
}

int ganlab_blur_bias_act_stats_f32(const float* x, const float* bias, const float* noise, const float* noise_w,
                                   float* y, float* mean, float* rstd, int N, int C, int H, int W, float bias_scale,
                                   int act, float slope, float eps, void* workspace, size_t workspace_bytes,
                                   void* stream) {
  if (!x || !y || !mean || !rstd || N <= 0 || C <= 0 || (noise && !noise_w)) return GANLAB_EINVAL;
  if (!ganlab_blur_fused_supported(H, W)) return GANLAB_EUNSUPPORTED;
  if (!workspace || workspace_bytes < ganlab_act_stats_workspace(N, C, (long long)H * W)) return GANLAB_EWORKSPACE;
  const int rows = blur_rows_mode(H, BF_FWD);
  long long per_n = (long long)(H / rows) * (W / 4);
  int chunks = (int)((per_n + 256 * 4 - 1) / (256 * 4));
  if (chunks < 1) chunks = 1;
  if (chunks > 128) chunks = 128;
  double* sp = reinterpret_cast<double*>(workspace);
  const dim3 grid((unsigned)chunks, (unsigned)C, (unsigned)N);
  if (rows == 8)
    GL_LAUNCH((blur_fused_kernel<BF_FWD, 8, true>), grid, dim3(256), 0, ST, x, (const float*)nullptr, noise, bias,
              noise_w, y, (double*)nullptr, N, C, H, W, chunks, bias_scale, act, slope, 0, sp);
  else if (rows == 4)
    GL_LAUNCH((blur_fused_kernel<BF_FWD, 4, true>), grid, dim3(256), 0, ST, x, (const float*)nullptr, noise, bias,
              noise_w, y, (double*)nullptr, N, C, H, W, chunks, bias_scale, act, slope, 0, sp);
  else
    GL_LAUNCH((blur_fused_kernel<BF_FWD, 2, true>), grid, dim3(256), 0, ST, x, (const float*)nullptr, noise, bias,
              noise_w, y, (double*)nullptr, N, C, H, W, chunks, bias_scale, act, slope, 0, sp);
  const long long planes = (long long)N * C;
  GL_LAUNCH(act_stats_finish_kernel, dim3((unsigned)((planes + 255) / 256)), dim3(256), 0, ST, (const double*)sp, mean,
            rstd, planes, chunks, 1.0 / ((double)H * W), eps);
  return GL_CHECK_LAUNCH();
}

int ganlab_blur_act_bwd_f32(const float* g, const float* y, float* out, float* gb, int N, int C, int H, int W,
                            float slope, float bias_scale, void* workspace, size_t workspace_bytes, void* stream) {
  if (!g || !y || !out || N <= 0 || C <= 0) return GANLAB_EINVAL;
  if (!ganlab_blur_fused_supported(H, W)) return GANLAB_EUNSUPPORTED;
  const int chunks = blur_fused_chunks(N, H, W);
  if (gb && (!workspace || workspace_bytes < (size_t)C * chunks * sizeof(double))) return GANLAB_EWORKSPACE;
  BLUR_FUSED_LAUNCH(BF_A, g, y, (const float*)nullptr, (const float*)nullptr, (const float*)nullptr, out,
                    (double*)workspace, N, C, H, W, chunks, 1.f, 0, slope, gb ? 1 : 0);
  if (gb) GL_LAUNCH(channel_sum_stage2, dim3(C), dim3(64), 0, ST, (const double*)workspace, gb, C, chunks, bias_scale);
  return GL_CHECK_LAUNCH();
}

int ganlab_blur_act_bwd_bits_f32(const float* g, const unsigned* ybits, float* out, float* gb, int N, int C, int H, int W,
                                 float slope, float bias_scale, void* workspace, size_t workspace_bytes, void* stream) {
  if (!g || !ybits || !out || N <= 0 || C <= 0) return GANLAB_EINVAL;
  if (!ganlab_blur_fused_supported(H, W) || !ganlab_mask_bits_supported(H, W)) return GANLAB_EUNSUPPORTED;
  const int chunks = blur_fused_chunks(N, H, W);
  if (gb && (!workspace || workspace_bytes < (size_t)C * chunks * sizeof(double))) return GANLAB_EWORKSPACE;
  BLUR_FUSED_LAUNCH_BITS(BF_A, g, reinterpret_cast<const float*>(ybits), (const float*)nullptr, (const float*)nullptr,
                         (const float*)nullptr, out, (double*)workspace, N, C, H, W, chunks, 1.f, 0, slope, gb ? 1 : 0);
  if (gb) GL_LAUNCH(channel_sum_stage2, dim3(C), dim3(64), 0, ST, (const double*)workspace, gb, C, chunks, bias_scale);
  return GL_CHECK_LAUNCH();
}

int ganlab_act_bwd_blur_bits_f32(const float* g, const unsigned* ybits, const float* noise, float* out, float* gb,
                                 float* gnw, int N, int C, int H, int W, float slope, float bias_scale, void* workspace,
                                 size_t workspace_bytes, void* stream) {
  if (!g || !ybits || !out || N <= 0 || C <= 0 || (gnw && !noise)) return GANLAB_EINVAL;
  if (!ganlab_blur_fused_supported(H, W) || !ganlab_mask_bits_supported(H, W)) return GANLAB_EUNSUPPORTED;
  const int chunks = blur_fused_chunks(N, H, W);
  const int sums = (gb || gnw) ? 1 : 0;
  if (sums && (!workspace || workspace_bytes < (size_t)2 * C * chunks * sizeof(double))) return GANLAB_EWORKSPACE;
  BLUR_FUSED_LAUNCH_BITS(BF_AT, g, reinterpret_cast<const float*>(ybits), gnw ? noise : (const float*)nullptr,
                         (const float*)nullptr, (const float*)nullptr, out, (double*)workspace, N, C, H, W, chunks, 1.f, 0,
                         slope, sums);
  if (gb) GL_LAUNCH(channel_sum_stage2, dim3(C), dim3(64), 0, ST, (const double*)workspace, gb, C, chunks, bias_scale);
  if (gnw)
    GL_LAUNCH(channel_sum_stage2, dim3(C), dim3(64), 0, ST, (const double*)workspace + (size_t)C * chunks, gnw, C,
              chunks, 1.f);
  return GL_CHECK_LAUNCH();
}

int ganlab_act_bwd_blur_f32(const float* g, const float* y, const float* noise, float* out, float* gb, float* gnw,
                            int N, int C, int H, int W, float slope, float bias_scale, void* workspace,
                            size_t workspace_bytes, void* stream) {
  if (!g || !y || !out || N <= 0 || C <= 0 || (gnw && !noise)) return GANLAB_EINVAL;
  if (!ganlab_blur_fused_supported(H, W)) return GANLAB_EUNSUPPORTED;
  const int chunks = blur_fused_chunks(N, H, W);
  const int sums = (gb || gnw) ? 1 : 0;
  if (sums && (!workspace || workspace_bytes < (size_t)2 * C * chunks * sizeof(double))) return GANLAB_EWORKSPACE;
  BLUR_FUSED_LAUNCH(BF_AT, g, y, gnw ? noise : (const float*)nullptr, (const float*)nullptr, (const float*)nullptr, out,
                    (double*)workspace, N, C, H, W, chunks, 1.f, 0, slope, sums);
  if (gb) GL_LAUNCH(channel_sum_stage2, dim3(C), dim3(64), 0, ST, (const double*)workspace, gb, C, chunks, bias_scale);
  if (gnw)
    GL_LAUNCH(channel_sum_stage2, dim3(C), dim3(64), 0, ST, (const double*)workspace + (size_t)C * chunks, gnw, C,
              chunks, 1.f);
  return GL_CHECK_LAUNCH();
}

int ganlab_instnorm_stats_f32(const float* x, float* mean, float* rstd, long long planes, long long HW, float eps,
                              void* stream) {
  if (!x || !mean || !rstd || planes <= 0 || HW <= 0) return GANLAB_EINVAL;
  const int vec = ((HW & 3) == 0 && (reinterpret_cast<uintptr_t>(x) & 15) == 0) ? 1 : 0;
  if (HW >= 1024)
    GL_LAUNCH(instnorm_stats_kernel<256>, dim3((unsigned)planes), dim3(256), 0, ST, x, mean, rstd, planes,
                       HW, eps, vec);
  else
    GL_LAUNCH(instnorm_stats_kernel<64>, dim3((unsigned)((planes + 3) / 4)), dim3(256), 0, ST, x, mean,
                       rstd, planes, HW, eps, vec);
  return GL_CHECK_LAUNCH();
}

size_t ganlab_row_stats_workspace(long long rows, long long M) {
  if (rows <= 0 || M <= 0) return 0;
  return (size_t)rows * act_stats_chunks(M / 4) * 2 * sizeof(double);
}

int ganlab_row_stats_f32(const float* x, float* mean, float* rstd, long long rows, long long M, float eps,
                         void* workspace, size_t workspace_bytes, void* stream) {
  if (!x || !mean || !rstd || rows <= 0 || M <= 0) return GANLAB_EINVAL;
  const int chunks = act_stats_chunks(M / 4);
  if ((M & 3) != 0 || chunks < 2 || rows * chunks > 0x7fffffffLL || (reinterpret_cast<uintptr_t>(x) & 15) != 0)
    return ganlab_instnorm_stats_f32(x, mean, rstd, rows, M, eps, stream);
  if (!workspace || workspace_bytes < ganlab_row_stats_workspace(rows, M)) return GANLAB_EWORKSPACE;
  double* sp = reinterpret_cast<double*>(workspace);
  GL_LAUNCH(row_stats_partial_kernel, dim3((unsigned)(rows * chunks)), dim3(256), 0, ST, x, sp, chunks, M >> 2);
  GL_LAUNCH(act_stats_finish_kernel, dim3((unsigned)((rows + 255) / 256)), dim3(256), 0, ST, (const double*)sp, mean,
            rstd, rows, chunks, 1.0 / (double)M, eps);
  return GL_CHECK_LAUNCH();
}

int ganlab_instnorm_style_fwd_f32(const float* x, const float* mean, const float* rstd, const float* style,
                                  float* y, int N, int C, long long HW, void* stream) {
  if (!x || !mean || !rstd || !y || N <= 0 || C <= 0 || HW <= 0) return GANLAB_EINVAL;
  static const int chunk_u = [] {
    const char* e = getenv("GANLAB_PW_CHUNK");
    const int v = e ? atoi(e) : 2;
    return (v == 0 || v == 2 || v == 4 || v == 8) ? v : 2;
  }();
  if (chunk_u > 0 && HW % (1024 * 8) == 0 && (long long)N * C * (HW / (1024 * chunk_u)) < 0x7fffffffLL) {
    const int chunks = (int)(HW / (1024 * chunk_u));
    const unsigned grid = (unsigned)((long long)N * C * chunks);
    if (chunk_u == 8) GL_LAUNCH(instnorm_style_fwd_chunk_kernel<8>, dim3(grid), dim3(256), 0, ST, x, mean, rstd, style, y, C, chunks, HW);
    else if (chunk_u == 2) GL_LAUNCH(instnorm_style_fwd_chunk_kernel<2>, dim3(grid), dim3(256), 0, ST, x, mean, rstd, style, y, C, chunks, HW);
    else GL_LAUNCH(instnorm_style_fwd_chunk_kernel<4>, dim3(grid), dim3(256), 0, ST, x, mean, rstd, style, y, C, chunks, HW);
  } else if ((HW & 3) == 0)
    GL_LAUNCH(instnorm_style_fwd_kernel<4>, dim3(ew_blocks((long long)N * C * HW / 4)), dim3(256), 0, ST,
                       x, mean, rstd, style, y, N, C, HW);
  else
    GL_LAUNCH(instnorm_style_fwd_kernel<1>, dim3(ew_blocks((long long)N * C * HW)), dim3(256), 0, ST, x,
                       mean, rstd, style, y, N, C, HW);
  return GL_CHECK_LAUNCH();
}

int ganlab_instnorm_style_bwd_reduce_f32(const float* gy, const float* x, const float* mean, const float* rstd,
                                         float* s1, float* s2, long long planes, long long HW, void* stream) {
  if (!gy || !x || !mean || !rstd || !s1 || !s2 || planes <= 0 || HW <= 0) return GANLAB_EINVAL;
  if (HW >= 1024)
    GL_LAUNCH(instnorm_bwd_reduce_kernel<256>, dim3((unsigned)planes), dim3(256), 0, ST, gy, x, mean,
                       rstd, s1, s2, planes, HW);
  else
    GL_LAUNCH(instnorm_bwd_reduce_kernel<64>, dim3((unsigned)((planes + 3) / 4)), dim3(256), 0, ST, gy, x,
                       mean, rstd, s1, s2, planes, HW);
  return GL_CHECK_LAUNCH();
}

int ganlab_instnorm_style_bwd_apply_f32(const float* gy, const float* x, const float* mean, const float* rstd,
                                        const float* style, const float* s1, const float* s2, float* gx, int N,
                                        int C, long long HW, void* stream) {
  if (!gy || !x || !mean || !rstd || !s1 || !s2 || !gx || N <= 0 || C <= 0 || HW <= 0) return GANLAB_EINVAL;
  if ((HW & 3) == 0)
    GL_LAUNCH(instnorm_bwd_apply_kernel<4>, dim3(ew_blocks((long long)N * C * HW / 4)), dim3(256), 0, ST,
                       gy, x, mean, rstd, style, s1, s2, gx, N, C, HW);
  else
    GL_LAUNCH(instnorm_bwd_apply_kernel<1>, dim3(ew_blocks((long long)N * C * HW)), dim3(256), 0, ST, gy,
                       x, mean, rstd, style, s1, s2, gx, N, C, HW);
  return GL_CHECK_LAUNCH();
}

int ganlab_pixelnorm_fwd_f32(const float* x, float* y, int N, int C, long long HW, float eps, void* stream) {
  if (!x || !y || N <= 0 || C <= 0 || HW <= 0) return GANLAB_EINVAL;
  const dim3 gd(ew_blocks((long long)N * HW)), bd(256);
  if (pixelnorm_generic()) GL_LAUNCH(pixelnorm_fwd_kernel, gd, bd, 0, ST, x, y, N, C, HW, eps);
  else if (C == 16) GL_LAUNCH(pixelnorm_fwd_reg_kernel<16>, gd, bd, 0, ST, x, y, N, HW, eps);
  else if (C == 32) GL_LAUNCH(pixelnorm_fwd_reg_kernel<32>, gd, bd, 0, ST, x, y, N, HW, eps);
  else if (C == 64) GL_LAUNCH(pixelnorm_fwd_reg_kernel<64>, gd, bd, 0, ST, x, y, N, HW, eps);
  else if (C == 128) GL_LAUNCH(pixelnorm_fwd_reg_kernel<128>, gd, bd, 0, ST, x, y, N, HW, eps);
  else if (pixelnorm_splits(N, C, HW) == 4)
    GL_LAUNCH(pixelnorm_fwd_split_kernel<4>, dim3(ew_blocks((long long)N * HW * 4)), bd, 0, ST, x, y, N, C, HW, eps);
  else if (pixelnorm_splits(N, C, HW) == 16)
    GL_LAUNCH(pixelnorm_fwd_split_kernel<16>, dim3(ew_blocks((long long)N * HW * 16)), bd, 0, ST, x, y, N, C, HW, eps);
  else GL_LAUNCH(pixelnorm_fwd_kernel, gd, bd, 0, ST, x, y, N, C, HW, eps);
  return GL_CHECK_LAUNCH();
}

int ganlab_pixelnorm_bwd_f32(const float* gy, const float* x, float* gx, int N, int C, long long HW, float eps,
                             void* stream) {
  if (!gy || !x || !gx || N <= 0 || C <= 0 || HW <= 0) return GANLAB_EINVAL;
  const dim3 gd(ew_blocks((long long)N * HW)), bd(256);
  if (pixelnorm_generic()) GL_LAUNCH(pixelnorm_bwd_kernel, gd, bd, 0, ST, gy, x, gx, N, C, HW, eps);
  else if (C == 16) GL_LAUNCH(pixelnorm_bwd_reg_kernel<16>, gd, bd, 0, ST, gy, x, gx, N, HW, eps);
  else if (C == 32) GL_LAUNCH(pixelnorm_bwd_reg_kernel<32>, gd, bd, 0, ST, gy, x, gx, N, HW, eps);
  else if (C == 64) GL_LAUNCH(pixelnorm_bwd_reg_kernel<64>, gd, bd, 0, ST, gy, x, gx, N, HW, eps);
  else if (C == 128) GL_LAUNCH(pixelnorm_bwd_reg_kernel<128>, gd, bd, 0, ST, gy, x, gx, N, HW, eps);
  else if (pixelnorm_splits(N, C, HW) == 4)
    GL_LAUNCH(pixelnorm_bwd_split_kernel<4>, dim3(ew_blocks((long long)N * HW * 4)), bd, 0, ST, gy, x, gx, N, C, HW, eps);
  else if (pixelnorm_splits(N, C, HW) == 16)
    GL_LAUNCH(pixelnorm_bwd_split_kernel<16>, dim3(ew_blocks((long long)N * HW * 16)), bd, 0, ST, gy, x, gx, N, C, HW,
              eps);
  else GL_LAUNCH(pixelnorm_bwd_kernel, gd, bd, 0, ST, gy, x, gx, N, C, HW, eps);
  return GL_CHECK_LAUNCH();
}

int ganlab_mbstd_fwd_f32(const float* x, float* stat, int G, int gs, long long F, float eps, void* stream) {
  if (!x || !stat || G <= 0 || gs <= 1 || F <= 0) return GANLAB_EINVAL;
  GL_LAUNCH(mbstd_fwd_kernel, dim3(G), dim3(256), 0, ST, x, stat, gs, F, eps);
  return GL_CHECK_LAUNCH();
}

int ganlab_mbstd_bwd_f32(const float* x, const float* gstat, float* gx, int G, int gs, long long F, float eps,
                         void* stream) {
  if (!x || !gstat || !gx || G <= 0 || gs <= 1 || F <= 0) return GANLAB_EINVAL;
  GL_LAUNCH(mbstd_bwd_kernel, dim3(ew_blocks((long long)G * F)), dim3(256), 0, ST, x, gstat, gx, G, gs, F,
                     eps);
  return GL_CHECK_LAUNCH();
}

int ganlab_mbstd_bwdbwd_f32(const float* x, const float* gstat, const float* ggx, float* g_gstat, float* g_x,
                            int G, int gs, long long F, float eps, void* stream) {
  if (!x || !gstat || !ggx || !g_gstat || !g_x || G <= 0 || gs <= 1 || F <= 0) return GANLAB_EINVAL;
  GL_LAUNCH(mbstd_bwdbwd_kernel, dim3(G), dim3(256), 0, ST, x, gstat, ggx, g_gstat, g_x, gs, F, eps);
  return GL_CHECK_LAUNCH();
}

int ganlab_chan_affine_f32(const float* x, const float* scale, const float* shift, float* y, int N, int C,
                           long long HW, void* stream) {
  if (!x || !y || N <= 0 || C <= 0 || HW <= 0) return GANLAB_EINVAL;
  if ((HW & 3) == 0 && ((reinterpret_cast<uintptr_t>(x) | reinterpret_cast<uintptr_t>(y)) & 15) == 0)
    GL_LAUNCH(chan_affine_kernel<4>, dim3(ew_blocks((long long)N * C * HW / 4)), dim3(256), 0, ST, x, scale, shift, y,
              N, C, HW);
  else
    GL_LAUNCH(chan_affine_kernel<1>, dim3(ew_blocks((long long)N * C * HW)), dim3(256), 0, ST, x, scale, shift, y, N,
              C, HW);
// ... 142 lines not shown
```

### gan_lab_amd/ops.py

```python
import collections
import ctypes
import os

import numpy as np

import torch
from torch.autograd import Function
from torch.autograd.function import once_differentiable

from . import _lib
from ._lib import ACT_LRELU, ACT_NONE, PACK_DGRAD, PACK_FWD, ConvGeom, check
from ._ops.core import (
    _p, _RAW_STREAM, _GET_DEVICE, _st, _c, _inplace, _same_numel, _gpu_device, _new, _ct, _aligned16, _nchw, _row_workspace,
    _INPUT_GRAD_ONLY, input_grad_only, _want_param_grads, _NO_GRAD_TOWARDS, no_grad_towards, _wants_input_grad, _DIRECT, _SINK,
    _TAKEN, _TAKE_HITS, direct_grads_enabled, direct_param_grads, _sink, _take, arena_takes, _sunk)
from ._ops.geom import (
    _COMPUTE, set_compute_dtype, get_compute_dtype, compute_dtype, Geom, pool_fusable, _OBSERVER, set_launch_observer, conv_flops,
    _note)
from ._ops.pointwise import (
    k_blur, decode_u8, k_up2, k_pool2, RESAMPLE_MODES, _RESAMPLE_TABLES, resample_matrix, _taps, _resample_tables, k_resample,
    k_bias_act, k_act_bwd, k_act_bwd_bias, k_channel_sum, k_axpby, k_scale_dev, k_sum, _ActBwd, _ActBwdBias, _ChanSum,
    _GroupBroadcast, _Blur, _Pool2, _Up2, _Resample, _Scale, _Axpby, _PixelNorm, _ChanAffine, _Mul, _Tanh, _TanhBwd, chan_affine,
    mul, tanh, channel_sum, blur, avg_pool2, upsample2, resample, lerp, scale, add, global_avg_pool, pixelnorm, group_broadcast)
from ._ops.norm import (
    _BatchNormTrain, batch_norm_composed, _ln_rowsums, _ln_project, _LayerNorm, _LayerNormBwd, layer_norm, layer_norm_composed)
from ._ops.loss import (
    _MbstdStat, _MbstdBwd, _Sum, _BceMean, _HingeMean, _HingeBwd, _ChNormPenalty, mbstd_stat, sum_all, sumsq_all, bce_logits_mean,
    hinge_mean, chnorm_penalty)
from ._ops.attention import (
    _ATTN_SECOND_ORDER, _attn_dims, attention_ok, k_attn_fwd, k_attn_bwd, _Attention, _AttentionBwd, _pool_dims, k_maxpool2x2,
    k_maxpool2x2_bwd, _MaxPool2x2, _MaxPool2x2Bwd, k_gated_residual, k_dot, _GatedResidual, _GatedResidualBwd, attention,
    max_pool2x2, gated_residual)
from ._ops.metrics import (
    SWD_DESC, _swd_planes, swd_down, swd_band, swd_gather, swd_stats, swd_project, _SWD_WS, _swd_workspace, swd_sort, swd_distance,
    swd_positions, swd_directions, PRDC_MAX_K, _prdc_rows, _prdc_vector, prdc_norms, prdc_knn, prdc_cross, MOMENTS_MAX_DIM,
    _accumulator, moments_accum, kid_rowsums, PPL_MAX_DIM, PPL_MODES, PPL_SAMPLINGS, PPL_RECORD, check_ppl_epsilon, ppl_endpoints,
    row_sqdist, trimmed_mean, MSSSIM_LEVELS, _msssim_images, msssim_workspace, msssim_level, msssim_finish,
    SPECTRUM_MIN_RES, SPECTRUM_MAX_RES, SPECTRUM_WINDOWS, _spectrum_size, spectrum_scratch_bytes, _spectrum_alloc,
    spectrum_workspace, spectrum_scratch, spectrum_feed, spectrum_finish)
from ._ops.optim import (
    SN_EPS, SnTable, sn_refresh, sn_backward, ortho_plan, OrthoTable, ortho_apply, lerp_rows, _adam_operands, adam_step,
    adam_step_dev, set_step_scalars, ewma_step, EwmaTable, ewma_many)
from ._ops.augment import (
    randn, check_truncation, trunc_randn, randn_dev, diffaug_params, diffaug_params_dev, k_diffaug, ADA_ROW, ADA_COUNTERS,
    ada_params, ada_params_dev, k_ada, ADA_EXT_ROW, ADA_EXT_COUNTERS, ADA_FILTER_TAPS, ADA_FILTER, ADA_NOISE, ADA_CUTOUT,
    ADA_NEW_GROUPS, AdaDraw, ada_filter_bank, ada_ext_params, ada_ext_params_dev, k_ada_ext, ada_update, _DiffAugment,
    _DiffAugmentAdjoint, _AdaAugment, _AdaAugmentAdjoint, diff_augment, ada_augment)
from ._ops.cond import _labels, randint, _bn_batch_stats, _CondBatchNorm, cond_batch_norm
from ._ops.hier import (
    _slot_open, HierTable, _HierModulate, hier_modulate, _ModBatchNorm, _mod_rows, _mod_stats, mod_batch_norm, mod_batch_norm_cols,
    _proj_dims, _ClassProj, _ClassProjDfeat, _ClassProjDweight, class_projection)
from ._ops.cr import (
    _cr_table, cr_params, cr_transform, _FirstOrderOnly, _first_order, _CrMsd, _cr_imsd_fwd, _CrImsd, _CrImsdHalves, cr_msd, cr_imsd)
from ._ops.cond_loss import (
    CL_MODES, CL_MAX_N, CL_MAX_E, CL_MAX_K, _cl_range, _ClassCrossEntropy, _ClassContrastive, class_cross_entropy, class_contrastive)
from ._ops.project import (
    PYRAMID_MAX_LEVELS, PROJECT_SCHEDULE, pyramid_max_levels, check_pyramid_weights, _PyramidMse, pyramid_mse, w_moments,
    check_project_schedule, project_step)


class _PackEntry(object):
    __slots__ = ('w', 'out', 'serial', 'ptr', 'row', 'desc')


_PACK_CACHE = {}
_PACK_SERIAL = [0]
_PACK_GEN = [0]
_PACK_RANGES = {}
_PACK_TABLES = {}
_KIND_PLAIN, _KIND_S2, _KIND_BF16, _KIND_X3 = 0, 1, 2, 3
BF16, X3, X3_UP, X3_DOWN, S2, LINEAR, F32 = 'bf16', 'x3', 'x3_up', 'x3_down', 's2', 'linear', 'f32'

_PackRow = collections.namedtuple('_PackRow', 'fn dtype args kind ks per_thread')
_PACK_ROWS = {
    F32: _PackRow('conv_pack_f32', torch.float32, ('ks', 'mode'), _KIND_PLAIN, None, None),
    S2: _PackRow('conv_s2_pack_f32', torch.float32, ('up', 'mode'), _KIND_S2, 3, 16),
    BF16: _PackRow('conv_pack_bf16', torch.bfloat16, ('mode',), _KIND_BF16, 3, 9),
    X3: _PackRow('conv_x3_pack', torch.bfloat16, ('mode',), _KIND_X3, 3, 27),
    X3_UP: _PackRow('conv_s2_x3_pack', torch.bfloat16, ('up',), _KIND_X3, 4, 48),
    X3_DOWN: _PackRow('conv_s2_down_x3_pack', torch.bfloat16, ('up',), _KIND_X3, 5, 48),
}


def bump_weight_epoch(ranges=None):
    _PACK_SERIAL[0] += 1
    if ranges is None:
        if _PACK_CACHE or _PACK_TABLES:
            _PACK_GEN[0] += 1
        _PACK_CACHE.clear()
        _PACK_TABLES.clear()
        _PACK_RANGES.clear()
        return
    for r in ranges:
        _PACK_RANGES[(int(r[0]), int(r[1]))] = _PACK_SERIAL[0]


def pack_generation():
    return _PACK_GEN[0]


_ALL_ADDRESSES = (0, 1 << 62)


def mark_packs_stale():
    if _PACK_RANGES:
        bump_weight_epoch(list(_PACK_RANGES.keys()))
    elif _PACK_CACHE:
        bump_weight_epoch([_ALL_ADDRESSES])


def _pack_call(row, w, out, desc, stream):
    _, cout, cin, ks, mode, up, scale, _ = desc
    args = {'ks': ks, 'mode': mode, 'up': up}
    return getattr(_lib.lib(), 'ganlab_' + row.fn)(_p(w), _p(out), cout, cin, *[args[a] for a in row.args], scale, stream)


def _pack_one(e):
    rc = _pack_call(e.row, e.w, e.out, e.desc, _st())
    if rc != e.desc[7]:
        raise _lib.GanlabLibraryError(f're-pack failed ({rc} != {e.desc[7]})')


def _stale_range(e):
    for r, ser in _PACK_RANGES.items():
        if ser > e.serial and r[0] <= e.ptr < r[1]:
            return r
    return None


def _repack_range(r):
    L = _lib.lib()
    ser = _PACK_RANGES[r]
    items = [(k, e) for k, e in _PACK_CACHE.items() if r[0] <= e.ptr < r[1] and e.serial < ser]
    keys = tuple(k for k, _ in items)
    tab = _PACK_TABLES.get(r)
    if (tab is None or tab[0] != keys) and torch.cuda.is_current_stream_capturing():
        for _, e in items:
            _pack_one(e)
            e.serial = _PACK_SERIAL[0]
        return
    if tab is None or tab[0] != keys:
        arr = (_lib.PackDesc * len(items))()
        blocks = 0
        for i, (_, e) in enumerate(items):
            kind, cout, cin, ks, mode, up, scale, total = e.desc
            d = arr[i]
            d.src, d.dst = e.w.data_ptr(), e.out.data_ptr()
            d.kind, d.Cout, d.Cin, d.ks, d.mode, d.up, d.scale, d.total, d.block0 = kind, cout, cin, ks, mode, up, scale, \
                total, blocks
            blocks += (total // (e.row.per_thread or ks * ks) + 255) // 256
        host = torch.frombuffer(bytearray(bytes(arr)), dtype=torch.uint8)
        if tab is not None:
            _PACK_GEN[0] += 1
        tab = (keys, host.to(items[0][1].w.device), blocks)
        _PACK_TABLES[r] = tab
    check(L.ganlab_pack_many(tab[1].data_ptr(), len(items), tab[2], _st()), 'pack_many')
    now = _PACK_SERIAL[0]
    for _, e in items:
        e.serial = now


def _pack_lookup(key):
    e = _PACK_CACHE.get(key)
    if e is None:
        return None
    r = _stale_range(e)
    if r is not None:
        _repack_range(r)
    return e.out


def _pack_store(key, w, out, row, desc):
    if len(_PACK_CACHE) > 1024:
# ... 1698 lines not shown
```

### include/ganlab_hip.h

```cpp
#ifndef GANLAB_HIP_H
#define GANLAB_HIP_H

#include <stddef.h>
#include <stdint.h>

#ifdef __cplusplus
extern "C" {
#endif

#define GANLAB_OK 0
#define GANLAB_EINVAL (-1)
#define GANLAB_EWORKSPACE (-2)
#define GANLAB_ELAUNCH (-3)
#define GANLAB_EUNSUPPORTED (-4)

#define GANLAB_ACT_NONE 0
#define GANLAB_ACT_LRELU 1

#define GANLAB_PACK_FWD 0
#define GANLAB_PACK_DGRAD 1

int ganlab_abi_version(void);

int ganlab_last_launch(char* name, int cap, unsigned* grid);
unsigned long long ganlab_launch_count(void);
int ganlab_launch_history(int back, char* name, int cap, unsigned* grid);

typedef struct {
  int N, Cin, Hin, Win;
  int Cout, ks, pad;
  int up;
  int pool;
} ganlab_conv_geom;

int ganlab_conv_geom_size(void);

int ganlab_conv_out_hw(const ganlab_conv_geom* g, int* Hout, int* Wout);

long long ganlab_conv_pack_f32(const float* w, float* out, int Cout, int Cin, int ks, int mode,
                               float scale, void* stream);

int ganlab_conv_fwd_f32(const float* x, const float* wp, const float* bias, float* y,
                        const ganlab_conv_geom* g, float bias_scale, int act, float slope,
                        void* stream);

int ganlab_conv_dgrad_f32(const float* gy, const float* wp, float* gx_virtual,
                          const ganlab_conv_geom* g, void* stream);

int ganlab_conv_splitk_plan(const ganlab_conv_geom* g, int dgrad);
int ganlab_conv_fwd_splitk_f32(const float* x, const float* wp, const float* bias, float* y, const ganlab_conv_geom* g,
                               float bias_scale, int act, float slope, void* workspace, size_t workspace_bytes,
                               void* stream);
int ganlab_conv_dgrad_splitk_f32(const float* gy, const float* wp, float* gx, const ganlab_conv_geom* g, void* workspace,
                                 size_t workspace_bytes, void* stream);

int ganlab_conv_dgrad_mask_supported(const ganlab_conv_geom* g);
int ganlab_conv_dgrad_mask_f32(const float* gy, const float* wp, const float* x, float* gx, const ganlab_conv_geom* g,
                               float slope, void* stream);

int ganlab_conv_act_bwd_fused_supported(const ganlab_conv_geom* g);
int ganlab_conv_dgrad_act_f32(const float* gy, const float* y, const float* wp, float* gx, const ganlab_conv_geom* g,
                              float slope, void* stream);
int ganlab_conv_fwd_mask_f32(const float* x, const float* wp, const float* y, float* out, const ganlab_conv_geom* g,
                             float slope, void* stream);
int ganlab_conv_wgrad_act_f32(const float* gy, const float* y, const float* x, float* gw, float* gb,
                              const ganlab_conv_geom* g, float scale, float bias_scale, float slope, void* workspace,
                              size_t workspace_bytes, void* stream);

size_t ganlab_conv_wgrad_workspace(const ganlab_conv_geom* g);
int ganlab_conv_wgrad_f32(const float* gy, const float* x, float* gw, const ganlab_conv_geom* g,
                          float scale, void* workspace, size_t workspace_bytes, void* stream);

int ganlab_conv_s2_supported(const ganlab_conv_geom* g);
long long ganlab_conv_s2_pack_f32(const float* w, float* out, int Cout, int Cin, int up, int transpose,
                                  float scale, void* stream);
int ganlab_conv_s2_fwd_f32(const float* x, const float* wp, const float* bias, float* y,
                           const ganlab_conv_geom* g, float bias_scale, int act, float slope, void* stream);
int ganlab_conv_s2_dgrad_f32(const float* gy, const float* wp, float* gx, const ganlab_conv_geom* g,
                             void* stream);
size_t ganlab_conv_s2_wgrad_workspace(const ganlab_conv_geom* g);
int ganlab_conv_s2_wgrad_f32(const float* gy, const float* x, float* gw, const ganlab_conv_geom* g,
                             float scale, void* workspace, size_t workspace_bytes, void* stream);

int ganlab_conv_bf16_supported(const ganlab_conv_geom* g);
long long ganlab_conv_pack_bf16(const float* w, void* out, int Cout, int Cin, int mode, float scale, void* stream);
int ganlab_conv_fwd_bf16(const float* x, const void* wp, const float* bias, float* y, const ganlab_conv_geom* g,
                         float bias_scale, int act, float slope, void* stream);
int ganlab_conv_dgrad_bf16(const float* gy, const void* wp, float* gx, const ganlab_conv_geom* g, void* stream);
int ganlab_conv_bf16_splitk_plan(const ganlab_conv_geom* g, int dgrad);
int ganlab_conv_fwd_bf16_splitk(const float* x, const void* wp, const float* bias, float* y, const ganlab_conv_geom* g,
                                float bias_scale, int act, float slope, void* workspace, size_t workspace_bytes,
                                void* stream);
int ganlab_conv_dgrad_bf16_splitk(const float* gy, const void* wp, float* gx, const ganlab_conv_geom* g, void* workspace,
                                  size_t workspace_bytes, void* stream);
size_t ganlab_conv_wgrad_bf16_workspace(const ganlab_conv_geom* g);
int ganlab_conv_wgrad_bf16(const float* gy, const float* x, float* gw, const ganlab_conv_geom* g, float scale,
                           void* workspace, size_t workspace_bytes, void* stream);

int ganlab_conv_x3_supported(const ganlab_conv_geom* g, int dgrad);
long long ganlab_conv_x3_pack(const float* w, void* out, int Cout, int Cin, int mode, float scale, void* stream);
int ganlab_conv_fwd_x3(const float* x, const void* wp, const float* bias, float* y, const ganlab_conv_geom* g,
                       float bias_scale, int act, float slope, void* stream);
int ganlab_conv_dgrad_x3(const float* gy, const void* wp, float* gx, const ganlab_conv_geom* g, void* stream);
int ganlab_conv_dgrad_mask_x3(const float* gy, const void* wp, const float* x, float* gx, const ganlab_conv_geom* g,
                              float slope, void* stream);
int ganlab_conv_fwd_aff_x3(const float* x, const void* wp, const float* aff_s, const float* aff_t, const float* bias,
                           float* y, const ganlab_conv_geom* g, float bias_scale, int act, float slope, void* stream);
int ganlab_conv_fwd_aff_tail_x3_chunks(const ganlab_conv_geom* g);
int ganlab_conv_s2_x3_supported(const ganlab_conv_geom* g, int dgrad);
long long ganlab_conv_s2_x3_pack(const float* w, void* out, int Cout, int Cin, int up, float scale, void* stream);
int ganlab_conv_s2_fwd_x3(const float* x, const void* wp, const float* bias, float* y, const ganlab_conv_geom* g,
                          float bias_scale, int act, float slope, void* stream);
int ganlab_conv_s2_fwd_aff_x3(const float* x, const void* wp, const float* aff_s, const float* aff_t, const float* bias,
                              float* y, const ganlab_conv_geom* g, float bias_scale, int act, float slope, void* stream);
int ganlab_conv_s2_dgrad_x3(const float* gy, const void* wp, float* gx, const ganlab_conv_geom* g, void* stream);
int ganlab_conv_s2_down_x3_supported(const ganlab_conv_geom* g, int dgrad);
long long ganlab_conv_s2_down_x3_pack(const float* w, void* out, int Cout, int Cin, int up, float scale, void* stream);
int ganlab_conv_s2_down_fwd_x3(const float* x, const void* wp, const float* bias, float* y, const ganlab_conv_geom* g,
                               float bias_scale, int act, float slope, void* stream);
int ganlab_conv_s2_down_dgrad_x3(const float* gy, const void* wp, float* gx, const ganlab_conv_geom* g, void* stream);
int ganlab_conv_wgrad_x3_supported(const ganlab_conv_geom* g);
size_t ganlab_conv_wgrad_x3_workspace(const ganlab_conv_geom* g);
int ganlab_conv_wgrad_x3(const float* gy, const float* x, const float* aff_s, const float* aff_t, float* gw,
                         const ganlab_conv_geom* g, float scale, void* workspace, size_t workspace_bytes, void* stream);
int ganlab_conv_s2_wgrad_x3_supported(const ganlab_conv_geom* g);
size_t ganlab_conv_s2_wgrad_x3_workspace(const ganlab_conv_geom* g);
int ganlab_conv_s2_wgrad_x3(const float* gy, const float* x, const float* aff_s, const float* aff_t, float* gw,
                            const ganlab_conv_geom* g, float scale, void* workspace, size_t workspace_bytes, void* stream);
int ganlab_conv_fwd_aff_tail_x3(const float* x, const void* wp, const float* aff_s, const float* aff_t, const float* bias,
                                const float* noise, const float* noise_w, float* y, float* mean, float* rstd,
                                const ganlab_conv_geom* g, float bias_scale, int act, float slope, float eps, void* workspace,
                                size_t workspace_bytes, void* stream);

int ganlab_blur3x3_f32(const float* x, float* y, long long planes, int H, int W, void* stream);
int ganlab_up2_f32(const float* x, float* y, long long planes, int H, int W, float scale, void* stream);
int ganlab_pool2_f32(const float* x, float* y, long long planes, int Hout, int Wout, float scale,
                     void* stream);
int ganlab_resample2d_f32(const float* x, float* y, const int* iy, const float* wy, const int* ix, const float* wx,
                          long long planes, int Hi, int Wi, int Ho, int Wo, int Ty, int Tx, void* stream);

int ganlab_bias_act_f32(const float* x, const float* bias, const float* noise, const float* noise_w,
                        float* y, int N, int C, long long HW, float bias_scale, int act, float slope,
                        void* stream);
int ganlab_act_bwd_f32(const float* gy, const float* y, float* gz, long long n, float slope, void* stream);
int ganlab_act_bwd_bias_f32(const float* gy, const float* y, float* gz, float* gb, int N, int C, long long HW,
                            float slope, float scale, void* workspace, size_t workspace_bytes, void* stream);
int ganlab_blur_fused_supported(int H, int W);
size_t ganlab_blur_fused_workspace(int N, int C, int H, int W);
int ganlab_blur_bias_act_f32(const float* x, const float* bias, const float* noise, const float* noise_w, float* y,
                             int N, int C, int H, int W, float bias_scale, int act, float slope, void* stream);
int ganlab_blur_act_bwd_f32(const float* g, const float* y, float* out, float* gb, int N, int C, int H, int W,
                            float slope, float bias_scale, void* workspace, size_t workspace_bytes, void* stream);
int ganlab_act_bwd_blur_f32(const float* g, const float* y, const float* noise, float* out, float* gb, float* gnw,
                            int N, int C, int H, int W, float slope, float bias_scale, void* workspace,
                            size_t workspace_bytes, void* stream);
size_t ganlab_act_stats_workspace(int N, int C, long long HW);
int ganlab_bias_act_stats_f32(const float* x, const float* bias, const float* noise, const float* noise_w, float* y,
                              float* mean, float* rstd, int N, int C, long long HW, float bias_scale, int act,
                              float slope, float eps, void* workspace, size_t workspace_bytes, void* stream);
int ganlab_blur_bias_act_stats_f32(const float* x, const float* bias, const float* noise, const float* noise_w,
                                   float* y, float* mean, float* rstd, int N, int C, int H, int W, float bias_scale,
                                   int act, float slope, float eps, void* workspace, size_t workspace_bytes,
                                   void* stream);
size_t ganlab_instnorm_bwd_act_workspace(int N, int C, long long HW);
int ganlab_instnorm_style_bwd_act_f32(const float* gy, const float* x, const float* mean, const float* rstd,
                                      const float* style, const float* s1, const float* s2, const float* noise,
                                      float* gz, float* gb, float* gnw, int N, int C, long long HW, int act,
                                      float slope, float bias_scale, void* workspace, size_t workspace_bytes,
                                      void* stream);
int ganlab_instnorm_style_bwd_act_blur_f32(const float* gy, const float* x, const float* mean, const float* rstd,
                                           const float* style, const float* s1, const float* s2, const float* noise,
                                           float* out, float* gb, float* gnw, int N, int C, int H, int W, int act,
                                           float slope, float bias_scale, void* workspace, size_t workspace_bytes,
                                           void* stream);
int ganlab_instnorm_bwd_rgb_supported(int N, int C, int crgb, long long HW);
size_t ganlab_instnorm_bwd_reduce_rgb_workspace(int N, int C, long long HW);
int ganlab_instnorm_style_bwd_reduce_rgb_f32(const float* grgb, const float* wp, int crgb, const float* x,
                                             const float* mean, const float* rstd, float* s1, float* s2, int N, int C,
                                             long long HW, void* workspace, size_t workspace_bytes, void* stream);
int ganlab_instnorm_style_bwd_act_rgb_f32(const float* grgb, const float* wp, int crgb, const float* x, const float* mean,
                                          const float* rstd, const float* style, const float* s1, const float* s2,
                                          const float* noise, float* gz, float* gb, float* gnw, int N, int C, long long HW,
                                          int act, float slope, float bias_scale, void* workspace, size_t workspace_bytes,
                                          void* stream);
int ganlab_channel_sum_f32(const float* a, const float* b_n1hw, float* out, int N, int C, long long HW,
                           float scale, void* workspace, size_t workspace_bytes, void* stream);
size_t ganlab_channel_sum_workspace(int N, int C, long long HW);

int ganlab_instnorm_stats_f32(const float* x, float* mean, float* rstd, long long planes, long long HW,
                              float eps, void* stream);
size_t ganlab_row_stats_workspace(long long rows, long long M);
int ganlab_row_stats_f32(const float* x, float* mean, float* rstd, long long rows, long long M, float eps,
                         void* workspace, size_t workspace_bytes, void* stream);
int ganlab_instnorm_style_fwd_f32(const float* x, const float* mean, const float* rstd,
                                  const float* style, float* y, int N, int C, long long HW, void* stream);
int ganlab_instnorm_style_bwd_reduce_f32(const float* gy, const float* x, const float* mean,
                                         const float* rstd, float* s1, float* s2, long long planes,
                                         long long HW, void* stream);
int ganlab_instnorm_style_bwd_apply_f32(const float* gy, const float* x, const float* mean,
                                        const float* rstd, const float* style, const float* s1,
                                        const float* s2, float* gx, int N, int C, long long HW,
                                        void* stream);
int ganlab_pixelnorm_fwd_f32(const float* x, float* y, int N, int C, long long HW, float eps, void* stream);
int ganlab_pixelnorm_bwd_f32(const float* gy, const float* x, float* gx, int N, int C, long long HW,
                             float eps, void* stream);

int ganlab_chan_affine_f32(const float* x, const float* scale, const float* shift, float* y, int N, int C,
                           long long HW, void* stream);
int ganlab_mul_f32(const float* a, const float* b, float* out, long long n, void* stream);
int ganlab_ln_affine_fwd_f32(const float* x, const float* mean, const float* rstd, const float* w, const float* b,
                             float* y, int N, long long M, int act, float slope, void* stream);
int ganlab_colscale_f32(const float* a, const float* w, float* out, int N, long long M, void* stream);
int ganlab_coldot_f32(const float* a, const float* x, const float* mean, const float* rstd, float* o1, float* o2,
                      int N, long long M, void* stream);
size_t ganlab_ln_rowsums_workspace(int N, long long M);
int ganlab_ln_rowsums_f32(const float* a, const float* wa, const float* x, const float* mean, const float* rstd,
                          const float* b2, const float* w2, float* out, int N, long long M, void* workspace,
                          size_t workspace_bytes, const float* yact, float* gz, float slope, void* stream);
int ganlab_ln_project_f32(const float* a, const float* wa, const float* x, const float* mean, const float* rstd,
                          const float* sums, const float* wo, float* out, int N, long long M, void* stream);
int ganlab_ln_bwd_cols_f32(const float* a, const float* w, const float* x, const float* mean, const float* rstd,
                           const float* sums, float* gx, float* gw, float* gb, int N, long long M, void* stream);
int ganlab_ln_bwdbwd_apply_f32(const float* x, const float* mean, const float* rstd, const float* pu, const float* gx,
                               const float* sums, const float* usums, float* out, int N, long long M, void* stream);
int ganlab_bn_stats_f32(const float* x, float* out, int N, int C, long long HW, void* workspace, size_t workspace_bytes,
                        void* stream);
int ganlab_bn_apply_f32(const float* x, const float* mean, const float* scale, const float* shift, float* y, int N,
                        int C, long long HW, int act, float slope, void* stream);
int ganlab_bn_finalize_f32(const float* mom, const float* weight, float* running_mean, float* running_var,
                           long long* batches, float* out, int C, float eps, float momentum, float unbias,
                           void* stream);
int ganlab_bn_bwd_sums_f32(const float* gy, const float* x, const float* mean, const float* rstd, float* out, int N,
                           int C, long long HW, void* workspace, size_t workspace_bytes, const float* yact, float* gz,
                           float slope, void* stream);
int ganlab_bn_bwd_apply_f32(const float* gy, const float* x, const float* mean, const float* rstd, const float* sums,
                            const float* pre, float* gx, int N, int C, long long HW, void* stream);
int ganlab_tanh_fwd_f32(const float* x, float* y, long long n, void* stream);
int ganlab_tanh_bwd_f32(const float* gy, const float* y, float* gx, long long n, void* stream);

int ganlab_mbstd_fwd_f32(const float* x, float* stat, int G, int gs, long long F, float eps, void* stream);
int ganlab_mbstd_bwd_f32(const float* x, const float* gstat, float* gx, int G, int gs, long long F,
                         float eps, void* stream);
int ganlab_mbstd_bwdbwd_f32(const float* x, const float* gstat, const float* ggx, float* g_gstat,
                            float* g_x, int G, int gs, long long F, float eps, void* stream);

int ganlab_axpby_f32(const float* x, const float* y, float* out, long long n, float a, float b, void* stream);
int ganlab_scale_dev_f32(const float* x, const float* gout, float* out, long long n, float a, void* stream);
int ganlab_lerp_rows_f32(const float* a, const float* b, const float* t, float* out, long long N, long long M,
                         void* stream);
int ganlab_sum_f32(const float* x, float* out, long long n, float scale, int squared, void* workspace,
                   size_t workspace_bytes, void* stream);
size_t ganlab_sum_workspace(long long n);
int ganlab_bce_logits_fwd_f32(const float* x, float* out, int n, float target, void* stream);
int ganlab_bce_logits_bwd_f32(const float* x, const float* gout, float* gx, int n, float target, void* stream);
int ganlab_hinge_fwd_f32(const float* x, float* out, int n, float a, float b, void* stream);
int ganlab_hinge_bwd_f32(const float* x, const float* gout, float* gx, int n, float a, float b, void* stream);
int ganlab_chnorm_penalty_fwd_f32(const float* g, float* out, int N, int C, long long HW, float gamma,
                                  float scale, void* workspace, size_t workspace_bytes, void* stream);
int ganlab_chnorm_penalty_bwd_f32(const float* g, const float* gout, float* gg, int N, int C, long long HW,
                                  float gamma, float scale, void* stream);

int ganlab_adam_f32(float* p, const float* g, float* m, float* v, long long n, float lr, float beta1,
                    float beta2, float eps, float wd, float bc1, float bc2, void* stream);
int ganlab_ewma_f32(float* lagged, const float* p, long long n, float beta, void* stream);
int ganlab_randn_f32(float* out, long long n, uint64_t seed, uint64_t offset, void* stream);

#define GANLAB_STEP_SCALARS_BYTES 64
int ganlab_step_scalars_size(void);
int ganlab_set_step_scalars(void* block, uint64_t rng_base, float f0, float f1, float f2, float f3, float f4, float f5,
                            void* stream);
int ganlab_randn_dev_f32(float* out, long long n, uint64_t seed, const void* base, uint64_t delta, void* stream);
int ganlab_adam_dev_f32(float* p, const float* g, float* m, float* v, long long n, const float* lr_bc1_bc2, float beta1,
                        float beta2, float eps, float wd, void* stream);


#define GANLAB_DIFFAUG_COLOR 1
#define GANLAB_DIFFAUG_TRANSLATION 2
#define GANLAB_DIFFAUG_CUTOUT 4
int ganlab_diffaug_params_f32(float* out, int N, int H, int W, uint64_t seed, uint64_t offset, void* stream);
int ganlab_diffaug_params_dev_f32(float* out, int N, int H, int W, uint64_t seed, const void* base, uint64_t delta,
                                  void* stream);
size_t ganlab_diffaug_fwd_workspace(int N, int H, int W, int policy);
size_t ganlab_diffaug_bwd_workspace(int N, int H, int W, int policy);
int ganlab_diffaug_fwd_f32(const float* x, const float* params, float* y, int N, int H, int W, int policy, void* workspace,
                           size_t workspace_bytes, void* stream);
int ganlab_diffaug_bwd_f32(const float* gy, const float* params, float* gx, int N, int H, int W, int policy,
                           void* workspace, size_t workspace_bytes, void* stream);

#define GANLAB_ADA_BLIT 1
#define GANLAB_ADA_GEOM 2
#define GANLAB_ADA_COLOR 4
#define GANLAB_ADA_ROW 32
#define GANLAB_ADA_COUNTERS 8
int ganlab_ada_params_f32(float* out, int N, int H, int W, const float* state, int policy, uint64_t seed, uint64_t offset,
                          void* stream);
int ganlab_ada_params_dev_f32(float* out, int N, int H, int W, const float* state, int policy, uint64_t seed,
                              const void* base, uint64_t delta, void* stream);
int ganlab_ada_fwd_f32(const float* x, const float* params, float* y, int N, int H, int W, void* stream);
int ganlab_ada_bwd_f32(const float* gy, const float* params, float* gx, int N, int H, int W, void* stream);
int ganlab_ada_update_f32(float* state, const float* logits, int N, int interval, float step_size, float target,
// ... 304 lines not shown
```

Before: 167.3 images/sec.

## Add row-streaming blur kernels that keep sliding 3-row window in registers

Adds streaming variants of the blur, fused blur+bias+act, blur backward, and instnorm-backward+blur kernels. Each wavefront walks a column strip down a segment of rows, keeping the horizontal partial sums of the previous two rows in registers and prefetching several rows at a time. This avoids re-reading halo rows per tile and aims at better memory-level parallelism. The variants are gated per family by image height through a runtime table set from Python, with an env var to disable them. The cost is more code paths, and the gates could pick the streaming path where it is slower.

```diff
diff --git a/gan_lab_amd/_lib.py b/gan_lab_amd/_lib.py
--- a/gan_lab_amd/_lib.py
+++ b/gan_lab_amd/_lib.py
@@ -177,6 +177,7 @@
     'ganlab_pixelnorm_fwd_f32': (_c_int, [_c_p, _c_p, _c_int, _c_int, _c_ll, _c_f, _c_p]),
     'ganlab_pixelnorm_bwd_f32': (_c_int, [_c_p, _c_p, _c_p, _c_int, _c_int, _c_ll, _c_f, _c_p]),
     'ganlab_blur_fused_supported': (_c_int, [_c_int, _c_int]),
+    'ganlab_set_blur_stream': (_c_int, [_c_int, _c_int, _c_int]),
     'ganlab_blur_fused_workspace': (_c_sz, [_c_int, _c_int, _c_int, _c_int]),
     'ganlab_blur_bias_act_f32': (_c_int, [_c_p, _c_p, _c_p, _c_p, _c_p, _c_int, _c_int, _c_int, _c_int, _c_f,
                                           _c_int, _c_f, _c_p]),
@@ -388,7 +389,18 @@
             raise GanlabLibraryError(f'EwmaJob mirror is {ctypes.sizeof(EwmaJob)} bytes, the library\'s '
                                      f'ganlab_ewma_job {handle.ganlab_ewma_job_size()}: header and binding disagree')
         _LIB = handle
+        for fn in _ON_LOAD:
+            fn(handle)
     return _LIB
+
+
+_ON_LOAD = []
+
+
+def on_load(fn):
+    _ON_LOAD.append(fn)
+    if _LIB is not None:
+        fn(_LIB)
 
 
 def last_launch():
diff --git a/gan_lab_amd/_ops/pointwise.py b/gan_lab_amd/_ops/pointwise.py
--- a/gan_lab_amd/_ops/pointwise.py
+++ b/gan_lab_amd/_ops/pointwise.py
@@ -1,3 +1,5 @@
+import os
+
 import numpy as np
 
 import torch
@@ -7,6 +9,34 @@
 from .. import _lib
 from .._lib import check
 from .core import _c, _nchw, _new, _p, _st, _take
+
+
+BLUR_STREAM_FAMILIES = ('blur', 'blur_bits', 'blur_bias_act', 'blur_bias_act_stats', 'blur_act_bwd', 'blur_act_bwd_bits',
+                        'act_bwd_blur', 'act_bwd_blur_bits', 'instnorm_bwd_act_blur')
+BLUR_STREAM_ROWS = 64
+BLUR_STREAM_GATE = {'blur': None, 'blur_bits': None, 'blur_bias_act': 256, 'blur_bias_act_stats': 256, 'blur_act_bwd': None,
+                    'blur_act_bwd_bits': None, 'act_bwd_blur': 256, 'act_bwd_blur_bits': 256, 'instnorm_bwd_act_blur': 512}
+_BLUR_STREAM = [1 if os.environ.get('GANLAB_BLUR_STREAM', '1') != '0' else 0]
+
+
+def _apply_blur_stream(handle, rows=None):
+    mode = _BLUR_STREAM[0]
+    for i, fam in enumerate(BLUR_STREAM_FAMILIES):
+        gate = BLUR_STREAM_GATE[fam]
+        min_h = -1 if (mode == 0 or (mode == 1 and gate is None)) else (gate if mode == 1 else 0)
+        check(handle.ganlab_set_blur_stream(i, min_h, rows or BLUR_STREAM_ROWS), 'set_blur_stream')
+
+
+_lib.on_load(_apply_blur_stream)
+
+
+def set_blur_stream(mode, rows=None):
+    mode = int(mode)
+    if mode not in (0, 1, 2):
+        raise ValueError(f'blur stream mode {mode!r}: 0, 1 or 2')
+    prev, _BLUR_STREAM[0] = _BLUR_STREAM[0], mode
+    _apply_blur_stream(_lib.lib(), rows)
+    return prev
 
 
 def k_blur(x):
diff --git a/gan_lab_amd/csrc/pointwise.hip b/gan_lab_amd/csrc/pointwise.hip
--- a/gan_lab_amd/csrc/pointwise.hip
+++ b/gan_lab_amd/csrc/pointwise.hip
@@ -65,6 +65,21 @@
 }
 __device__ __forceinline__ unsigned mask_bit(const unsigned* __restrict__ bits, long long e) {
   return (bits[e >> 5] >> (unsigned)(e & 31)) & 1u;
+}
+
+__device__ __forceinline__ void blur_row_combine(float4 v, float e, int q, int w4, float (&hrow)[4], float (&cen)[4]) {
+  const int lane = threadIdx.x & 63;
+  float l = __shfl_up(v.w, 1, 64);
+  float r = __shfl_down(v.x, 1, 64);
+  if (q == 0) l = 0.f;
+  else if (lane == 0) l = e;
+  if (q == w4 - 1) r = 0.f;
+  else if (lane == 63) r = e;
+  hrow[0] = l + 2.f * v.x + v.y;
+  hrow[1] = v.x + 2.f * v.y + v.z;
+  hrow[2] = v.y + 2.f * v.z + v.w;
+  hrow[3] = v.z + 2.f * v.w + r;
+  cen[0] = v.x; cen[1] = v.y; cen[2] = v.z; cen[3] = v.w;
 }
 
 template <bool MASKED, bool BITS = false>
@@ -92,8 +107,6 @@
     }
   }
   const int lane = threadIdx.x & 63;
-  float l = __shfl_up(v.w, 1, 64);
-  float r = __shfl_down(v.x, 1, 64);
   const bool need_l = lane == 0 && q != 0, need_r = lane == 63 && q != w4 - 1;
   float e = 0.f;
   if (valid && (need_l || need_r)) {
@@ -104,15 +117,7 @@
       else e = m[eo] > 0.f ? e : e * slope;
     }
   }
-  if (q == 0) l = 0.f;
-  else if (lane == 0) l = e;
-  if (q == w4 - 1) r = 0.f;
-  else if (lane == 63) r = e;
-  hrow[0] = l + 2.f * v.x + v.y;
-  hrow[1] = v.x + 2.f * v.y + v.z;
-  hrow[2] = v.y + 2.f * v.z + v.w;
-  hrow[3] = v.z + 2.f * v.w + r;
-  cen[0] = v.x; cen[1] = v.y; cen[2] = v.z; cen[3] = v.w;
+  blur_row_combine(v, e, q, w4, hrow, cen);
 }
 
 template <int R, bool BITS = false>
@@ -412,7 +417,9 @@
 #define BLUR_FUSED_LAUNCH(MODE, ...)                                                                   \
   do {                                                                                                 \
     const int rows_ = blur_rows_mode(H, MODE);                                                         \
-    if (rows_ == 8) GL_LAUNCH((blur_fused_kernel<MODE, 8>), dim3(chunks, C), dim3(256), 0, ST, __VA_ARGS__);      \
+    if (stream_)                                                                                       \
+      GL_LAUNCH((blur_fused_stream_kernel<MODE>), dim3(chunks, C), dim3(256), 0, ST, __VA_ARGS__, (double*)nullptr, stream_); \
+    else if (rows_ == 8) GL_LAUNCH((blur_fused_kernel<MODE, 8>), dim3(chunks, C), dim3(256), 0, ST, __VA_ARGS__);      \
     else if (rows_ == 4) GL_LAUNCH((blur_fused_kernel<MODE, 4>), dim3(chunks, C), dim3(256), 0, ST, __VA_ARGS__); \
     else GL_LAUNCH((blur_fused_kernel<MODE, 2>), dim3(chunks, C), dim3(256), 0, ST, __VA_ARGS__);                \
   } while (0)
@@ -420,10 +427,342 @@
 #define BLUR_FUSED_LAUNCH_BITS(MODE, ...)                                                                            \
   do {                                                                                                               \
     const int rows_ = blur_rows_mode(H, MODE);                                                                       \
-    if (rows_ == 8) GL_LAUNCH((blur_fused_kernel<MODE, 8, false, true>), dim3(chunks, C), dim3(256), 0, ST, __VA_ARGS__);      \
+    if (stream_)                                                                                                     \
+      GL_LAUNCH((blur_fused_stream_kernel<MODE, false, true>), dim3(chunks, C), dim3(256), 0, ST, __VA_ARGS__,             \
+                (double*)nullptr, stream_);                                                                                \
+    else if (rows_ == 8) GL_LAUNCH((blur_fused_kernel<MODE, 8, false, true>), dim3(chunks, C), dim3(256), 0, ST, __VA_ARGS__);      \
     else if (rows_ == 4) GL_LAUNCH((blur_fused_kernel<MODE, 4, false, true>), dim3(chunks, C), dim3(256), 0, ST, __VA_ARGS__); \
     else GL_LAUNCH((blur_fused_kernel<MODE, 2, false, true>), dim3(chunks, C), dim3(256), 0, ST, __VA_ARGS__);                \
   } while (0)
+
+constexpr int STRIP_P = 4;
+
+struct StripRow {
+  float4 v, m, nz;
+  unsigned nbw, ebw;
+  float e, em;
+};
+
+__device__ __forceinline__ float4 ld4(const float* p) { return *reinterpret_cast<const float4*>(p); }
+
+template <class F, class G>
+__device__ __forceinline__ void strip_walk(int r0, int r1, F&& fetch, G&& step) {
+  for (int yb = r0 - 1; yb <= r1; yb += STRIP_P) {
+    StripRow raw[STRIP_P];
+#pragma unroll
+    for (int k = 0; k < STRIP_P; ++k) fetch(yb + k, raw[k]);
+#pragma unroll
+    for (int k = 0; k < STRIP_P; ++k) step(yb + k, raw[k]);
+  }
+}
+
+__device__ __forceinline__ int strip_edge_offset(int lane, int q, int w4) {
+  return (lane == 0 && q != 0) ? -1 : ((lane == 63 && q != w4 - 1) ? 4 : 0);
+}
+
+__device__ __forceinline__ unsigned sign_nibble(const float (&c)[4]) {
+  return (c[0] > 0.f ? 1u : 0u) | (c[1] > 0.f ? 2u : 0u) | (c[2] > 0.f ? 4u : 0u) | (c[3] > 0.f ? 8u : 0u);
+}
+
+template <bool BITS>
+__global__ __launch_bounds__(256) void blur3x3_stream_kernel(const float* __restrict__ x, float* __restrict__ y, int planes,
+                                                             int H, int W, int S, unsigned* __restrict__ bits) {
+  const int strips = W >> 8, w4 = W >> 2, nseg = (H + S - 1) / S;
+  const int lane = threadIdx.x & 63;
+  const int u = gl_xcd_remap(blockIdx.x, gridDim.x) * 4 + (threadIdx.x >> 6);
+  if (u >= planes * strips * nseg) return;
+  const int seg = u % nseg, t = u / nseg, strip = t % strips, pl = t / strips;
+  const long long plane = (long long)pl * H * W;
+  const int q = strip * 64 + lane, x0 = 4 * q, eoff = strip_edge_offset(lane, q, w4);
+  const int r0 = seg * S, r1 = min(r0 + S, H);
+  const float* px = x + plane + x0;
+  float* py = y + plane + x0;
+  float hm[4] = {0.f, 0.f, 0.f, 0.f}, h0[4] = {0.f, 0.f, 0.f, 0.f};
+  auto fetch = [&](int row, StripRow& r) {
+    const int ro = min(max(row, 0), H - 1) * W;
+    r.v = ld4(px + ro);
+    r.e = px[ro + eoff];
+  };
+  auto step = [&](int row, const StripRow& r) {
+    const bool valid = (unsigned)row < (unsigned)H;
+    const float4 v = valid ? r.v : make_float4(0.f, 0.f, 0.f, 0.f);
+    float hn[4], cen[4];
+    blur_row_combine(v, valid ? r.e : 0.f, q, w4, hn, cen);
+    if constexpr (BITS) {
+      if (row >= r0 && row < r1) {
+        unsigned wv = sign_nibble(cen) << (4 * (lane & 7));
+        wv |= __shfl_xor(wv, 1, 64);
+        wv |= __shfl_xor(wv, 2, 64);
+        wv |= __shfl_xor(wv, 4, 64);
+        if ((lane & 7) == 0) bits[(plane + (long long)row * W + x0) >> 5] = wv;
+      }
+    }
+    if (row > r0 && row <= r1) {
+      float4 o;
+      o.x = (hm[0] + 2.f * h0[0] + hn[0]) * 0.0625f;
+      o.y = (hm[1] + 2.f * h0[1] + hn[1]) * 0.0625f;
+      o.z = (hm[2] + 2.f * h0[2] + hn[2]) * 0.0625f;
+      o.w = (hm[3] + 2.f * h0[3] + hn[3]) * 0.0625f;
+      *reinterpret_cast<float4*>(py + (row - 1) * W) = o;
+    }
+#pragma unroll
+    for (int j = 0; j < 4; ++j) { hm[j] = h0[j]; h0[j] = hn[j]; }
+  };
+  strip_walk(r0, r1, fetch, step);
+}
+
+template <int MODE, bool STATS = false, bool BITS = false>
+__global__ __launch_bounds__(256) void blur_fused_stream_kernel(const float* __restrict__ in, const float* __restrict__ y,
+                                                                const float* __restrict__ noise,
+                                                                const float* __restrict__ bias,
+                                                                const float* __restrict__ noise_w,
+                                                                float* __restrict__ out, double* __restrict__ part, int N,
+                                                                int C, int H, int W, int chunks, float bias_scale, int act,
+                                                                float slope, int want_sums, double* __restrict__ spart,
+                                                                int S) {
+  __shared__ double red[4];
+  __shared__ double dred[2][4];
+  int id = gl_xcd_remap((int)(blockIdx.x + gridDim.x * (blockIdx.y + gridDim.y * blockIdx.z)),
+                        (int)(gridDim.x * gridDim.y * gridDim.z));
+  const int chunk = id % chunks;
+  id /= chunks;
+  const int c = id % C, img = id / C;
+  const int strips = W >> 8, w4 = W >> 2, nseg = (H + S - 1) / S;
+  const int units = (STATS ? 1 : N) * strips * nseg, per = (units + chunks * 4 - 1) / (chunks * 4);
+  const int lane = threadIdx.x & 63;
+  const int HW = H * W;
+  const unsigned* mb = reinterpret_cast<const unsigned*>(y);
+  const bool has_nz = noise && (MODE == BF_FWD || (MODE == BF_AT && want_sums));
+  double ds = 0.0, dss = 0.0;
+  const float b = (MODE == BF_FWD && bias) ? bias[c] * bias_scale : 0.f;
+  const float nw = (MODE == BF_FWD && noise) ? noise_w[c] : 0.f;
+  double s0 = 0.0, s1 = 0.0;
+  const int ubeg = (chunk * 4 + (int)(threadIdx.x >> 6)) * per, uend = min(ubeg + per, units);
+  for (int u = ubeg; u < uend; ++u) {
+    const int seg = u % nseg, t = u / nseg, strip = t % strips, n = STATS ? img : t / strips;
+    const long long plane = ((long long)n * C + c) * HW;
+    const int q = strip * 64 + lane, x0 = 4 * q, eoff = strip_edge_offset(lane, q, w4);
+    const int r0 = seg * S, r1 = min(r0 + S, H);
+    const float* pin = in + plane + x0;
+    const float* pm = (MODE != BF_FWD && !BITS) ? y + plane + x0 : pin;
+    const unsigned* pw = BITS ? mb + ((plane + x0) >> 5) : nullptr;
+    const unsigned* pwe = BITS ? mb + ((plane + x0 + eoff) >> 5) : nullptr;
+    const unsigned sh = (unsigned)(x0 & 31), she = (unsigned)((x0 + eoff) & 31);
+    const float* pn = has_nz ? noise + (long long)n * HW + x0 : pin;
+    float* po = out + plane + x0;
+    float hm[4] = {0.f, 0.f, 0.f, 0.f}, h0[4] = {0.f, 0.f, 0.f, 0.f}, nz0[4] = {0.f, 0.f, 0.f, 0.f};
+    unsigned nib0 = 0;
+    auto fetch = [&](int row, StripRow& r) {
+      const int ro = min(max(row, 0), H - 1) * W;
+      r.v = ld4(pin + ro);
+      r.e = pin[ro + eoff];
+      if (MODE != BF_FWD) {
+        if (BITS) {
+          r.nbw = pw[ro >> 5];
+          if (MODE == BF_AT) r.ebw = pwe[ro >> 5];
+        } else {
+          r.m = ld4(pm + ro);
+          if (MODE == BF_AT) r.em = pm[ro + eoff];
+        }
+      }
+      if (MODE != BF_A) r.nz = ld4(pn + ro);
+    };
+    auto step = [&](int row, const StripRow& r) {
+      const bool valid = (unsigned)row < (unsigned)H, own = row >= r0 && row < r1;
+      float4 v = r.v;
+      float e = r.e;
+      unsigned nib = 0;
+      if (MODE != BF_FWD) {
+        if (BITS) nib = (r.nbw >> sh) & 0xFu;
+        else nib = (r.m.x > 0.f ? 1u : 0u) | (r.m.y > 0.f ? 2u : 0u) | (r.m.z > 0.f ? 4u : 0u) | (r.m.w > 0.f ? 8u : 0u);
+      }
+      if (MODE == BF_AT) {
+        v.x = (nib & 1u) ? v.x : v.x * slope;
+        v.y = (nib & 2u) ? v.y : v.y * slope;
+        v.z = (nib & 4u) ? v.z : v.z * slope;
+        v.w = (nib & 8u) ? v.w : v.w * slope;
+        const bool epos = BITS ? ((r.ebw >> she) & 1u) != 0u : r.em > 0.f;
+        e = epos ? e : e * slope;
+      }
+      if (!valid) {
+        v = make_float4(0.f, 0.f, 0.f, 0.f);
+        e = 0.f;
+      }
+      float hn[4], cen[4], nzn[4] = {0.f, 0.f, 0.f, 0.f};
+      blur_row_combine(v, e, q, w4, hn, cen);
+      if (MODE != BF_A && has_nz) { nzn[0] = r.nz.x; nzn[1] = r.nz.y; nzn[2] = r.nz.z; nzn[3] = r.nz.w; }
+      if (MODE == BF_AT && own) {
+#pragma unroll
+        for (int j = 0; j < 4; ++j) {
+          s0 += (double)cen[j];
+          s1 += (double)cen[j] * nzn[j];
+        }
+      }
+      if (row > r0 && row <= r1) {
+        float o[4];
+#pragma unroll
+        for (int j = 0; j < 4; ++j) o[j] = (hm[j] + 2.f * h0[j] + hn[j]) * 0.0625f;
+        if (MODE == BF_FWD) {
+#pragma unroll
+          for (int j = 0; j < 4; ++j) {
+            float t = o[j] + b + nw * nz0[j];
+            if (act == GANLAB_ACT_LRELU) t = gl_lrelu(t, slope);
+            o[j] = t;
+            if (STATS) {
+              const double d = (double)t;
+              ds += d;
+              dss += d * d;
+            }
+          }
+        } else if (MODE == BF_A) {
+#pragma unroll
+          for (int j = 0; j < 4; ++j) {
+            o[j] = ((nib0 >> j) & 1u) ? o[j] : o[j] * slope;
+            s0 += (double)o[j];
+          }
+        }
+        *reinterpret_cast<float4*>(po + (row - 1) * W) = *reinterpret_cast<float4*>(o);
+      }
+#pragma unroll
+      for (int j = 0; j < 4; ++j) { hm[j] = h0[j]; h0[j] = hn[j]; nz0[j] = nzn[j]; }
+      nib0 = nib;
+    };
+    strip_walk(r0, r1, fetch, step);
+  }
+  if (STATS) {
+#pragma unroll
+    for (int o = 32; o > 0; o >>= 1) {
+      ds += __shfl_xor(ds, o, 64);
+      dss += __shfl_xor(dss, o, 64);
+    }
+    if ((threadIdx.x & 63) == 0) {
+      dred[0][threadIdx.x >> 6] = ds;
+      dred[1][threadIdx.x >> 6] = dss;
+    }
+    __syncthreads();
+    if (threadIdx.x < 2) {
+      const int k = threadIdx.x;
+      spart[(((long long)img * C + c) * chunks + chunk) * 2 + k] = (dred[k][0] + dred[k][1]) + (dred[k][2] + dred[k][3]);
+    }
+  }
+  if (MODE != BF_FWD && want_sums) {
+    s0 = gl_block_sum_256d(s0, red);
+    if (threadIdx.x == 0) part[(long long)c * chunks + chunk] = s0;
+    if (MODE == BF_AT) {
+      __syncthreads();
+      s1 = gl_block_sum_256d(s1, red);
+      if (threadIdx.x == 0) part[((long long)C + c) * chunks + chunk] = s1;
+    }
+  }
+}
+
+__global__ __launch_bounds__(256) void instnorm_bwd_act_blur_stream_kernel(
+    const float* __restrict__ gy, const float* __restrict__ x, const float* __restrict__ mean,
+    const float* __restrict__ rstd, const float* __restrict__ style, const float* __restrict__ s1,
+    const float* __restrict__ s2, const float* __restrict__ noise, float* __restrict__ out, double* __restrict__ part,
+    int N, int C, int H, int W, int chunks, int S, int act, float slope, int want_b, int want_nw) {
+  __shared__ double red[4];
+  int id = gl_xcd_remap((int)(blockIdx.x + gridDim.x * (blockIdx.y + gridDim.y * blockIdx.z)),
+                        (int)(gridDim.x * gridDim.y * gridDim.z));
+  const int chunk = id % chunks;
+  id /= chunks;
+  const int c = id % C, n = id / C;
+  const int HW = H * W;
+  const long long pl = (long long)n * C + c;
+  const int strips = W >> 8, w4 = W >> 2, nseg = (H + S - 1) / S;
+  const int units = strips * nseg, per = (units + chunks * 4 - 1) / (chunks * 4);
+  const double md = (double)mean[pl], rd = (double)rstd[pl];
+  const double ys = style ? (double)style[((long long)n * 2 + 0) * C + c] + 1.0 : 1.0;
+  const double inv = 1.0 / (double)HW;
+  const double k = rd * ys, a1 = (double)s1[pl] * inv, a2 = (double)s2[pl] * inv;
+  const bool has_nz = want_nw && noise;
+  const int lane = threadIdx.x & 63;
+  double sb = 0.0, snw = 0.0;
+  auto zval = [&](float g, float v) -> double {
+    double t = k * ((double)g - a1 - ((double)v - md) * rd * a2);
+    if (act == GANLAB_ACT_LRELU && !(v > 0.f)) t *= (double)slope;
+    return t;
+  };
+  const int ubeg = (chunk * 4 + (int)(threadIdx.x >> 6)) * per, uend = min(ubeg + per, units);
+  for (int u = ubeg; u < uend; ++u) {
+    const int seg = u % nseg, strip = u / nseg;
+    const int q = strip * 64 + lane, x0 = 4 * q, eoff = strip_edge_offset(lane, q, w4);
+    const int r0 = seg * S, r1 = min(r0 + S, H);
+    const float* pg = gy + pl * HW + x0;
+    const float* px = x + pl * HW + x0;
+    const float* pn = has_nz ? noise + (long long)n * HW + x0 : pg;
+    float* po = out + pl * HW + x0;
+    float hm[4] = {0.f, 0.f, 0.f, 0.f}, h0[4] = {0.f, 0.f, 0.f, 0.f};
+    auto fetch = [&](int row, StripRow& r) {
+      const int ro = min(max(row, 0), H - 1) * W;
+      r.v = ld4(pg + ro);
+      r.m = ld4(px + ro);
+      r.e = pg[ro + eoff];
+      r.em = px[ro + eoff];
+      r.nz = ld4(pn + ro);
+    };
+    auto step = [&](int row, const StripRow& r) {
+      const bool valid = (unsigned)row < (unsigned)H, own = row >= r0 && row < r1;
+      const float g[4] = {r.v.x, r.v.y, r.v.z, r.v.w}, v[4] = {r.m.x, r.m.y, r.m.z, r.m.w};
+      const float nz[4] = {r.nz.x, r.nz.y, r.nz.z, r.nz.w};
+      float z[4];
+#pragma unroll
+      for (int j = 0; j < 4; ++j) {
+        const double t = zval(g[j], v[j]);
+        z[j] = valid ? (float)t : 0.f;
+        if (own) {
+          sb += t;
+          snw += t * (double)(has_nz ? nz[j] : 0.f);
+        }
+      }
+      const float e = valid ? (float)zval(r.e, r.em) : 0.f;
+      float hn[4], cen[4];
+      blur_row_combine(make_float4(z[0], z[1], z[2], z[3]), e, q, w4, hn, cen);
+      if (row > r0 && row <= r1) {
+        float4 o;
+        o.x = (hm[0] + 2.f * h0[0] + hn[0]) * 0.0625f;
+        o.y = (hm[1] + 2.f * h0[1] + hn[1]) * 0.0625f;
+        o.z = (hm[2] + 2.f * h0[2] + hn[2]) * 0.0625f;
+        o.w = (hm[3] + 2.f * h0[3] + hn[3]) * 0.0625f;
+        *reinterpret_cast<float4*>(po + (row - 1) * W) = o;
+      }
+#pragma unroll
+      for (int j = 0; j < 4; ++j) { hm[j] = h0[j]; h0[j] = hn[j]; }
+    };
+    strip_walk(r0, r1, fetch, step);
+  }
+  const long long slot = ((long long)c * N + n) * chunks + chunk;
+  if (want_b) {
+    sb = gl_block_sum_256d(sb, red);
+    if (threadIdx.x == 0) part[slot] = sb;
+  }
+  if (want_nw) {
+    if (want_b) __syncthreads();
+    snw = gl_block_sum_256d(snw, red);
+    if (threadIdx.x == 0) part[(long long)C * N * chunks + slot] = snw;
+  }
+}
+
+enum { BS_BLUR = 0, BS_BLUR_BITS, BS_FWD, BS_FWD_STATS, BS_A, BS_A_BITS, BS_AT, BS_AT_BITS, BS_INORM, BS_COUNT };
+struct BlurStreamGate { int min_h, rows; };
+BlurStreamGate g_blur_stream[BS_COUNT] = {{0x7fffffff, 32}, {0x7fffffff, 32}, {0x7fffffff, 32}, {0x7fffffff, 32}, {0x7fffffff, 32},
+                                          {0x7fffffff, 32}, {0x7fffffff, 32}, {0x7fffffff, 32}, {0x7fffffff, 32}};
+
+inline int blur_stream_rows(int family, long long domain, long long blocks, int H, int W) {
+  const BlurStreamGate g = g_blur_stream[family];
+  if ((W & 255) != 0 || H < 2 || H < g.min_h || (long long)H * W >= 0x7fffffffLL) return 0;
+  const long long units = domain * (W >> 8) * ((H + g.rows - 1) / g.rows);
+  if (units >= 0x1fffffffLL || blocks >= 0x7fffffffLL) return 0;
+  return g.rows;
+}
+inline int blur_stream_plane_chunks(int H, int W, int S, int cap) {
+  const int c = ((W >> 8) * ((H + S - 1) / S) + 3) / 4;
+  return c < 1 ? 1 : (c > cap ? cap : c);
+}
+
+inline unsigned blur_stream_blocks(long long planes, int H, int W, int S) {
+  return (unsigned)((planes * (W >> 8) * ((H + S - 1) / S) + 3) / 4);
+}
 
 inline int blur_fused_chunks(int N, int H, int W) {
   long long c = ((long long)N * (H / blur_rows(H)) * (W / 4) + 256 * 4 - 1) / (256 * 4);
@@ -1533,7 +1872,10 @@
 int ganlab_blur3x3_f32(const float* x, float* y, long long planes, int H, int W, void* stream) {
   if (!x || !y || planes <= 0 || H <= 0 || W <= 0) return GANLAB_EINVAL;
   if ((W & 3) == 0 && (H & 1) == 0 && ((reinterpret_cast<uintptr_t>(x) | reinterpret_cast<uintptr_t>(y)) & 15) == 0)
-    if ((H & 7) == 0 && H >= 256)
+    if (const int S = blur_stream_rows(BS_BLUR, planes, planes * (W >> 8) * (H / 2 + 1), H, W))
+      GL_LAUNCH(blur3x3_stream_kernel<false>, dim3(blur_stream_blocks(planes, H, W, S)), dim3(256), 0, ST, x, y, (int)planes, H,
+                W, S, (unsigned*)nullptr);
+    else if ((H & 7) == 0 && H >= 256)
       GL_LAUNCH(blur3x3_vec_kernel<8>, dim3(ew_blocks(planes * (H / 8) * (W / 4))), dim3(256), 0, ST, x, y, planes, H,
                 W);
     else if ((H & 3) == 0)
@@ -1553,7 +1895,10 @@
   if (!x || !y || !bits || planes <= 0) return GANLAB_EINVAL;
   if (!ganlab_mask_bits_supported(H, W) || ((reinterpret_cast<uintptr_t>(x) | reinterpret_cast<uintptr_t>(y)) & 15) != 0)
     return GANLAB_EUNSUPPORTED;
-  if ((H & 7) == 0 && H >= 256)
+  if (const int S = blur_stream_rows(BS_BLUR_BITS, planes, planes * (W >> 8) * (H / 2 + 1), H, W))
+    GL_LAUNCH(blur3x3_stream_kernel<true>, dim3(blur_stream_blocks(planes, H, W, S)), dim3(256), 0, ST, x, y, (int)planes, H, W,
+              S, bits);
+  else if ((H & 7) == 0 && H >= 256)
     GL_LAUNCH((blur3x3_vec_kernel<8, true>), dim3(ew_blocks(planes * (H / 8) * (W / 4))), dim3(256), 0, ST, x, y, planes, H,
               W, bits);
   else if ((H & 3) == 0)
@@ -1630,6 +1975,16 @@
   return GL_CHECK_LAUNCH();
 }
 
+int ganlab_set_blur_stream(int family, int min_h, int seg_rows) {
+  if (family < -1 || family >= BS_COUNT || seg_rows < 2 || seg_rows > 4096) return GANLAB_EINVAL;
+  for (int f = 0; f < BS_COUNT; ++f)
+    if (family == -1 || family == f) {
+      g_blur_stream[f].min_h = min_h < 0 ? 0x7fffffff : min_h;
+      g_blur_stream[f].rows = seg_rows;
+    }
+  return GANLAB_OK;
+}
+
 int ganlab_blur_fused_supported(int H, int W) { return (H >= 2 && W >= 4 && (H & 1) == 0 && (W & 3) == 0) ? 1 : 0; }
 
 size_t ganlab_blur_fused_workspace(int N, int C, int H, int W) {
@@ -1642,6 +1997,7 @@
   if (!x || !y || N <= 0 || C <= 0 || (noise && !noise_w)) return GANLAB_EINVAL;
   if (!ganlab_blur_fused_supported(H, W)) return GANLAB_EUNSUPPORTED;
   const int chunks = blur_fused_chunks(N, H, W);
+  const int stream_ = blur_stream_rows(BS_FWD, N, (long long)chunks * C, H, W);
   BLUR_FUSED_LAUNCH(BF_FWD, x, (const float*)nullptr, noise, bias, noise_w, y, (double*)nullptr, N, C, H, W, chunks,
                     bias_scale, act, slope, 0);
   return GL_CHECK_LAUNCH();
@@ -1755,9 +2111,14 @@
   int chunks = (int)((per_n + 256 * 4 - 1) / (256 * 4));
   if (chunks < 1) chunks = 1;
   if (chunks > 64) chunks = 64;
+  const int S = blur_stream_rows(BS_INORM, 1, 64LL * C * N, H, W);
+  if (S) chunks = blur_stream_plane_chunks(H, W, S, 64);
   double* part = reinterpret_cast<double*>(workspace);
   const dim3 grid((unsigned)chunks, (unsigned)C, (unsigned)N);
-  if (rows == 4)
+  if (S)
+    GL_LAUNCH(instnorm_bwd_act_blur_stream_kernel, grid, dim3(256), 0, ST, gy, x, mean, rstd, style, s1, s2, noise, out, part,
+              N, C, H, W, chunks, S, act, slope, gb ? 1 : 0, gnw ? 1 : 0);
+  else if (rows == 4)
     GL_LAUNCH(instnorm_bwd_act_blur_kernel<4>, grid, dim3(256), 0, ST, gy, x, mean, rstd, style, s1, s2, noise, out, part, N, C,
               H, W, chunks, act, slope, gb ? 1 : 0, gnw ? 1 : 0);
   else
@@ -1798,9 +2159,14 @@
   int chunks = (int)((per_n + 256 * 4 - 1) / (256 * 4));
   if (chunks < 1) chunks = 1;
   if (chunks > 128) chunks = 128;
+  const int S = blur_stream_rows(BS_FWD_STATS, 1, 128LL * C * N, H, W);
+  if (S) chunks = blur_stream_plane_chunks(H, W, S, 128);
   double* sp = reinterpret_cast<double*>(workspace);
   const dim3 grid((unsigned)chunks, (unsigned)C, (unsigned)N);
-  if (rows == 8)
+  if (S)
+    GL_LAUNCH((blur_fused_stream_kernel<BF_FWD, true>), grid, dim3(256), 0, ST, x, (const float*)nullptr, noise, bias,
+              noise_w, y, (double*)nullptr, N, C, H, W, chunks, bias_scale, act, slope, 0, sp, S);
+  else if (rows == 8)
     GL_LAUNCH((blur_fused_kernel<BF_FWD, 8, true>), grid, dim3(256), 0, ST, x, (const float*)nullptr, noise, bias,
               noise_w, y, (double*)nullptr, N, C, H, W, chunks, bias_scale, act, slope, 0, sp);
   else if (rows == 4)
@@ -1821,6 +2187,7 @@
   if (!ganlab_blur_fused_supported(H, W)) return GANLAB_EUNSUPPORTED;
   const int chunks = blur_fused_chunks(N, H, W);
   if (gb && (!workspace || workspace_bytes < (size_t)C * chunks * sizeof(double))) return GANLAB_EWORKSPACE;
+  const int stream_ = blur_stream_rows(BS_A, N, (long long)chunks * C, H, W);
   BLUR_FUSED_LAUNCH(BF_A, g, y, (const float*)nullptr, (const float*)nullptr, (const float*)nullptr, out,
                     (double*)workspace, N, C, H, W, chunks, 1.f, 0, slope, gb ? 1 : 0);
   if (gb) GL_LAUNCH(channel_sum_stage2, dim3(C), dim3(64), 0, ST, (const double*)workspace, gb, C, chunks, bias_scale);
@@ -1833,6 +2200,7 @@
   if (!ganlab_blur_fused_supported(H, W) || !ganlab_mask_bits_supported(H, W)) return GANLAB_EUNSUPPORTED;
   const int chunks = blur_fused_chunks(N, H, W);
   if (gb && (!workspace || workspace_bytes < (size_t)C * chunks * sizeof(double))) return GANLAB_EWORKSPACE;
+  const int stream_ = blur_stream_rows(BS_A_BITS, N, (long long)chunks * C, H, W);
   BLUR_FUSED_LAUNCH_BITS(BF_A, g, reinterpret_cast<const float*>(ybits), (const float*)nullptr, (const float*)nullptr,
                          (const float*)nullptr, out, (double*)workspace, N, C, H, W, chunks, 1.f, 0, slope, gb ? 1 : 0);
   if (gb) GL_LAUNCH(channel_sum_stage2, dim3(C), dim3(64), 0, ST, (const double*)workspace, gb, C, chunks, bias_scale);
@@ -1847,6 +2215,7 @@
   const int chunks = blur_fused_chunks(N, H, W);
   const int sums = (gb || gnw) ? 1 : 0;
   if (sums && (!workspace || workspace_bytes < (size_t)2 * C * chunks * sizeof(double))) return GANLAB_EWORKSPACE;
+  const int stream_ = blur_stream_rows(BS_AT_BITS, N, (long long)chunks * C, H, W);
   BLUR_FUSED_LAUNCH_BITS(BF_AT, g, reinterpret_cast<const float*>(ybits), gnw ? noise : (const float*)nullptr,
                          (const float*)nullptr, (const float*)nullptr, out, (double*)workspace, N, C, H, W, chunks, 1.f, 0,
                          slope, sums);
@@ -1865,6 +2234,7 @@
   const int chunks = blur_fused_chunks(N, H, W);
   const int sums = (gb || gnw) ? 1 : 0;
   if (sums && (!workspace || workspace_bytes < (size_t)2 * C * chunks * sizeof(double))) return GANLAB_EWORKSPACE;
+  const int stream_ = blur_stream_rows(BS_AT, N, (long long)chunks * C, H, W);
   BLUR_FUSED_LAUNCH(BF_AT, g, y, gnw ? noise : (const float*)nullptr, (const float*)nullptr, (const float*)nullptr, out,
                     (double*)workspace, N, C, H, W, chunks, 1.f, 0, slope, sums);
   if (gb) GL_LAUNCH(channel_sum_stage2, dim3(C), dim3(64), 0, ST, (const double*)workspace, gb, C, chunks, bias_scale);
diff --git a/gan_lab_amd/ops.py b/gan_lab_amd/ops.py
--- a/gan_lab_amd/ops.py
+++ b/gan_lab_amd/ops.py
@@ -18,7 +18,7 @@
     _COMPUTE, set_compute_dtype, get_compute_dtype, compute_dtype, Geom, pool_fusable, _OBSERVER, set_launch_observer, conv_flops,
     _note)
 from ._ops.pointwise import (
-    k_blur, decode_u8, k_up2, k_pool2, RESAMPLE_MODES, _RESAMPLE_TABLES, resample_matrix, _taps, _resample_tables, k_resample,
+    BLUR_STREAM_FAMILIES, BLUR_STREAM_GATE, set_blur_stream, k_blur, decode_u8, k_up2, k_pool2, RESAMPLE_MODES, _RESAMPLE_TABLES, resample_matrix, _taps, _resample_tables, k_resample,
     k_bias_act, k_act_bwd, k_act_bwd_bias, k_channel_sum, k_axpby, k_scale_dev, k_sum, _ActBwd, _ActBwdBias, _ChanSum,
     _GroupBroadcast, _Blur, _Pool2, _Up2, _Resample, _Scale, _Axpby, _PixelNorm, _ChanAffine, _Mul, _Tanh, _TanhBwd, chan_affine,
     mul, tanh, channel_sum, blur, avg_pool2, upsample2, resample, lerp, scale, add, global_avg_pool, pixelnorm, group_broadcast)
diff --git a/include/ganlab_hip.h b/include/ganlab_hip.h
--- a/include/ganlab_hip.h
+++ b/include/ganlab_hip.h
@@ -146,6 +146,7 @@
 int ganlab_act_bwd_bias_f32(const float* gy, const float* y, float* gz, float* gb, int N, int C, long long HW,
                             float slope, float scale, void* workspace, size_t workspace_bytes, void* stream);
 int ganlab_blur_fused_supported(int H, int W);
+int ganlab_set_blur_stream(int family, int min_h, int seg_rows);
 size_t ganlab_blur_fused_workspace(int N, int C, int H, int W);
 int ganlab_blur_bias_act_f32(const float* x, const float* bias, const float* noise, const float* noise_w, float* y,
                              int N, int C, int H, int W, float bias_scale, int act, float slope, void* stream);
```

After: 167.4 images/sec (median of 5 runs). No clear change (+0.1%).
